# MaartenGr/PolyFuzz

Hardware: AMD Instinct MI355X
Metric: string-pairs/sec, TF-IDF cosine top-n 100k x 100k (config.timed_step says what a step is: by default the user-level .match() call of SURVEY section 8d's metric, `device_step` = the list resident in HBM; latency.top1_single_query_ms = top-1 match latency) (higher is better)
Workload: dtype f32

## Files before the change

### polyfuzz_amd/csrc/k1_vectorize.hip

```cpp
#include "pfz_internal.h"

#include <string.h>

#include <algorithm>
#include <atomic>
#include <type_traits>

namespace pfz {

constexpr uint32_t kInvalid = 0xFFFFFFFFu;
constexpr int kShortMax = 128;
constexpr int kLongMax = 4096;
constexpr int kLongTile = 16;
constexpr int kMaxCodeBits = 64;
constexpr int kBitmapMaxBits = 32;

static std::atomic<uint64_t> g_gen{1};

struct VocabView {
    const uint32_t *bitmap;
    const int32_t *prefix;
    const uint64_t *vcodes;
    int64_t vocab;
};
// ... 503 lines not shown
    df[k] = s;
}

constexpr int kHistRows = 1024;

__global__ __launch_bounds__(1024) void k_df_hist(const int64_t *__restrict__ off, int64_t n, int32_t R,
                                                   const uint64_t *__restrict__ slots,
                                                   const int32_t *__restrict__ row_nnz, int32_t words,
                                                   uint32_t *__restrict__ partial, ListB B = ListB{})
{
    __shared__ uint32_t h[kHistWords];
    for (int t = threadIdx.x; t < words; t += 1024) h[t] = 0u;
    __syncthreads();
    unsigned bx = blockIdx.x;
    if (bx >= B.grid0) {
        bx -= B.grid0;
        off = B.off;
        n = B.n;
        slots = B.slots;
        row_nnz = B.row_cnt + (B.n + 1);
    }
    const int64_t r0 = (int64_t)bx * kHistRows;
    const int64_t r1 = r0 + kHistRows < n ? r0 + kHistRows : n;
    const int grp = threadIdx.x >> 4, sub = threadIdx.x & 15;
    const int lane0 = (threadIdx.x & 63) & ~15;
    for (int64_t rb = r0 + grp * 16; rb < r1; rb += 64 * 16) {
        const int64_t mine = rb + sub;
        int nn = 0;
        int64_t so = 0;
        if (mine < r1) {
            nn = row_nnz[mine];
            so = off[mine] * R;
        }
        uint32_t kk[16];
        int nni[16];
#pragma unroll
        for (int i = 0; i < 16; ++i) {
            nni[i] = __shfl(nn, lane0 + i, 64);
            const int64_t soi = ((int64_t)__shfl((int)(so >> 32), lane0 + i, 64) << 32) |
                                (uint32_t)__shfl((int)(uint32_t)so, lane0 + i, 64);
            kk[i] = sub < nni[i] ? ((const uint2 *)(slots + soi))[sub].x : 0u;
        }
#pragma unroll
        for (int i = 0; i < 16; ++i)
            if (sub < nni[i]) atomicAdd(&h[kk[i] >> 1], 1u << ((kk[i] & 1u) * 16));
        for (int i = 0; i < 16; ++i) {
            const int n_i = __shfl(nn, lane0 + i, 64);
            if (n_i <= 16) continue;
            const int64_t soi = ((int64_t)__shfl((int)(so >> 32), lane0 + i, 64) << 32) |
                                (uint32_t)__shfl((int)(uint32_t)so, lane0 + i, 64);
            const uint2 *in = (const uint2 *)(slots + soi);
            for (int t = sub + 16; t < n_i; t += 16) {
                const uint32_t k = in[t].x;
                atomicAdd(&h[k >> 1], 1u << ((k & 1u) * 16));
            }
        }
    }
    __syncthreads();
    uint32_t *dst = partial + (int64_t)blockIdx.x * words;
    for (int t = threadIdx.x; t < words; t += 1024) dst[t] = h[t];
}

__global__ __launch_bounds__(256) void k_df_hist_reduce(const uint32_t *__restrict__ partial, int32_t words,
                                                         int32_t chunks, int64_t vocab, int32_t *__restrict__ df,
                                                         double n_docs = 0.0, double *__restrict__ idf = nullptr)
{
    const int w = blockIdx.x * 256 + threadIdx.x;
    if (w >= words) return;
    int32_t lo = 0, hi = 0;
#pragma unroll 8
    for (int c = 0; c < chunks; ++c) {
        const uint32_t v = partial[(int64_t)c * words + w];
        lo += (int32_t)(v & 0xffffu);
        hi += (int32_t)(v >> 16);
    }
    df[2 * (int64_t)w] = lo;
    if (2 * (int64_t)w + 1 < vocab) df[2 * (int64_t)w + 1] = hi;
    if (idf) {
        idf[2 * (int64_t)w] = log((n_docs + 1.0) / ((double)lo + 1.0)) + 1.0;
        if (2 * (int64_t)w + 1 < vocab) idf[2 * (int64_t)w + 1] = log((n_docs + 1.0) / ((double)hi + 1.0)) + 1.0;
    }
}

__global__ __launch_bounds__(256) void k_rows_short(const int64_t *__restrict__ off, int64_t n, int32_t R,
                                                     VocabView V, uint64_t *__restrict__ slots,
                                                     const int32_t *__restrict__ row_cnt,
                                                     int32_t *__restrict__ row_nnz, DfSink df, ListB B = ListB{})
{
    const int lane = threadIdx.x & 63;
    unsigned bx = blockIdx.x;
    if (bx >= B.grid0) {
        bx -= B.grid0;
        off = B.off;
        n = B.n;
        slots = B.slots;
        row_cnt = B.row_cnt;
        row_nnz = B.row_cnt + (B.n + 1);
    }
    const int64_t row = (int64_t)bx * 4 + (threadIdx.x >> 6);
    if (row >= n) return;
    const int cnt = row_cnt[row];
    if (cnt > kShortMax) return;
    if (cnt == 0) {
        if (lane == 0) row_nnz[row] = 0;
        return;
    }
    rows_short_row(V, slots + off[row] * R, cnt, lane, row_nnz + row, row, df);
}

template <typename KEYS>
__device__ inline void rows_long_body(KEYS keys, int cnt, const VocabView &V, uint64_t *base, int32_t *row_nnz_out,
                                      DfSink df, int *sh_heads, int *sh_valid)
{
    const int lane = threadIdx.x & 63, wave = threadIdx.x >> 6;
    int npow2 = 128;
    while (npow2 < cnt) npow2 <<= 1;
    for (int t = threadIdx.x; t < npow2; t += 256) keys[t] = t < cnt ? vocab_rank(V, base[t]) : kInvalid;
    __syncthreads();
    for (int k = 2; k <= npow2; k <<= 1) {
        for (int j = k >> 1; j > 0; j >>= 1) {
            for (int t = threadIdx.x; t < npow2; t += 256) {
                const int x = t ^ j;
                if (x > t) {
                    const bool asc = (t & k) == 0;
                    const uint32_t a = keys[t], b = keys[x];
                    if ((a > b) == asc) {
                        keys[t] = b;
                        keys[x] = a;
                    }
                }
            }
            __syncthreads();
        }
    }
    uint2 *out = (uint2 *)base;
    if (wave == 0) {
        int nheads = 0, nvalid = 0;
        for (int c0 = 0; c0 < cnt; c0 += 64) {
            const int t = c0 + lane;
            uint32_t key = kInvalid, prev = kInvalid;
            if (t < cnt) key = keys[t];
            if (t > 0 && t < cnt) prev = keys[t - 1];
            const bool valid = key != kInvalid;
            const bool head = valid && (t == 0 || key != prev);
            const uint64_t H = __ballot(head);
            if (head) {
                out[nheads + __popcll(H & ((1ull << lane) - 1ull))] = make_uint2(key, (uint32_t)t);
                df.add(key, blockIdx.x);
            }
            nheads += __popcll(H);
            nvalid += __popcll(__ballot(valid));
        }
        if (lane == 0) {
            *sh_heads = nheads;
            *sh_valid = nvalid;
            *row_nnz_out = nheads;
        }
    }
    __syncthreads();
    const int nheads = *sh_heads, nvalid = *sh_valid;
    for (int c0 = 0; c0 < nheads; c0 += 256) {
        const int p = c0 + threadIdx.x;
        uint32_t tf = 0;
        if (p < nheads) tf = (p + 1 < nheads ? out[p + 1].y : (uint32_t)nvalid) - out[p].y;
        __syncthreads();
        if (p < nheads) out[p].y = tf;
        __syncthreads();
    }
}

__global__ __launch_bounds__(256) void k_rows_long(const int64_t *__restrict__ off, int64_t n, int32_t R, VocabView V,
                                                    uint64_t *__restrict__ slots,
                                                    const int32_t *__restrict__ row_cnt,
                                                    int32_t *__restrict__ row_nnz, DfSink df,
                                                    uint32_t *__restrict__ giant_scratch, int64_t giant_stride)
{
    __shared__ uint32_t lds_keys[kLongMax];
    __shared__ int sh_heads, sh_valid, n_long;
    __shared__ int long_rows[kLongTile];
    const int64_t n_tiles = (n + kLongTile - 1) / kLongTile;
    for (int64_t tile = blockIdx.x; tile < n_tiles; tile += gridDim.x) {
        if (threadIdx.x == 0) n_long = 0;
        __syncthreads();
        const int64_t mine = tile * kLongTile + threadIdx.x;
        if ((int)threadIdx.x < kLongTile && mine < n && row_cnt[mine] > kShortMax) long_rows[atomicAdd(&n_long, 1)] = (int)threadIdx.x;
        __syncthreads();
        const int m = n_long;
        for (int i = 0; i < m; ++i) {
            const int64_t row = tile * kLongTile + long_rows[i];
            const int cnt = row_cnt[row];
            uint64_t *base = slots + off[row] * R;
            if (cnt <= kLongMax)
                rows_long_body(&lds_keys[0], cnt, V, base, row_nnz + row, df, &sh_heads, &sh_valid);
            else
                rows_long_body(giant_scratch + (int64_t)blockIdx.x * giant_stride, cnt, V, base, row_nnz + row, df,
                               &sh_heads, &sh_valid);
            __syncthreads();
        }
        __syncthreads();
    }
}

__global__ __launch_bounds__(256) void k_idf(const int32_t *__restrict__ df, int64_t vocab, double n_docs,
                                              double *__restrict__ idf)
{
    const int64_t k = (int64_t)blockIdx.x * 256 + threadIdx.x;
    if (k >= vocab) return;
    idf[k] = log((n_docs + 1.0) / ((double)df[k] + 1.0)) + 1.0;
}

__device__ inline double shfl_f64(double v, int src_lane)
{
    const int lo = __shfl(__double2loint(v), src_lane, 64), hi = __shfl(__double2hiint(v), src_lane, 64);
    return __hiloint2double(hi, lo);
}

constexpr int64_t kSelfScanRows = 16384;
template <bool SELF_SCAN>
__global__ __launch_bounds__(256) void k_finalize(const int64_t *__restrict__ off, int64_t n, int32_t R,
                                                   const uint64_t *__restrict__ slots,
                                                   int32_t *__restrict__ indptr, const double *__restrict__ idf,
                                                   int32_t *__restrict__ indices, float *__restrict__ data,
                                                   const int32_t *__restrict__ row_nnz, int32_t *__restrict__ host_total)
{
    const int64_t row = ((int64_t)blockIdx.x * 256 + threadIdx.x) >> 4;
    const int sub = threadIdx.x & 15;
    const int lane0 = (threadIdx.x & 63) & ~15;
    const bool live = row < n;
    const uint2 *in = live ? (const uint2 *)(slots + off[row] * R) : nullptr;
    int o, nn;
    if (SELF_SCAN) {
        __shared__ int32_t s_part[4], s_cnt[16];
        const int64_t row0 = (int64_t)blockIdx.x * 16;
        int32_t acc = 0;
        for (int64_t t = threadIdx.x; t < row0; t += 256) acc += row_nnz[t];
        for (int d = 32; d >= 1; d >>= 1) acc += __shfl_xor(acc, d, 64);
        if ((threadIdx.x & 63) == 0) s_part[threadIdx.x >> 6] = acc;
        if (threadIdx.x < 16) s_cnt[threadIdx.x] = row0 + threadIdx.x < n ? row_nnz[row0 + threadIdx.x] : 0;
        __syncthreads();
        o = s_part[0] + s_part[1] + s_part[2] + s_part[3];
        const int mine = (int)(row - row0);
        for (int k = 0; k < mine; ++k) o += s_cnt[k];
        nn = live ? s_cnt[mine] : 0;
        if (live && sub == 0) indptr[row] = o;
        if (row == n - 1 && sub == 0) {
            indptr[n] = o + nn;
            if (host_total) __hip_atomic_store(host_total, o + nn, __ATOMIC_RELAXED, __HIP_MEMORY_SCOPE_SYSTEM);
        }
    } else {
        o = live ? indptr[row] : 0;
        nn = live ? indptr[row + 1] - o : 0;
    }
    int nn_max = nn;
    for (int d = 16; d < 64; d <<= 1) nn_max = max(nn_max, __shfl_xor(nn_max, d, 64));
    double ss = 0.0;
    for (int c0 = 0; c0 < nn_max; c0 += 16) {
        const int t = c0 + sub;
        double v = 0.0;
        if (t < nn) {
            const uint2 e = in[t];
            v = __dmul_rn((double)e.y, idf[e.x]);
        }
        const double v2 = __dmul_rn(v, v);
        const int m = min(16, nn_max - c0);
        for (int j = 0; j < m; ++j) {
            const double term = shfl_f64(v2, lane0 + j);
            if (c0 + j < nn) ss = __dadd_rn(ss, term);
        }
    }
    const double nrm = sqrt(ss);
    for (int t = sub; t < nn; t += 16) {
        const uint2 e = in[t];
        double v = __dmul_rn((double)e.y, idf[e.x]);
        if (ss != 0.0) v = v / nrm;
        indices[o + t] = (int32_t)e.x;
        data[o + t] = (float)v;
    }
}

__global__ __launch_bounds__(256) void k_copy_i32(const int32_t *__restrict__ src, int64_t n, int32_t *__restrict__ dst)
{
    const int64_t i = (int64_t)blockIdx.x * 256 + threadIdx.x;
    if (i < n) dst[i] = src[i];
}

static inline unsigned grid_for(int64_t n, int per_block = 256) { return (unsigned)((n + per_block - 1) / per_block); }

static int bits_for(uint64_t max_value)
{
    int b = 1;
    while ((max_value >> b) != 0) ++b;
    return b;
}

static int prepare_slots(pfz_ctx *ctx, const pfz_tfidf *v, pfz_strings *s)
{
    const int R = v->params.ngram_hi - v->params.ngram_lo + 1;
    const size_t need = (size_t)(s->n_units > 0 ? s->n_units : 1) * (size_t)R;
    if (s->slots_cap < need) {
        if (s->slots) pool_free(s->slots);
        s->slots = nullptr;
        PFZ_TRY(pool_alloc(ctx, &s->slots, need * sizeof(uint64_t)));
        s->slots_cap = need;
    }
    if (!s->row_cnt) PFZ_TRY(pool_alloc(ctx, &s->row_cnt, (size_t)(s->n + 1) * 2 * sizeof(int32_t)));
    return PFZ_OK;
}

static int run_extract(pfz_ctx *ctx, const pfz_tfidf *v, pfz_strings *s, bool mark, bool *rows_done = nullptr,
                       pfz_strings *sb = nullptr, bool *sb_done = nullptr)
{
    if (sb_done) *sb_done = false;
    PFZ_TRY(prepare_slots(ctx, v, s));
    if (s->n == 0) return PFZ_OK;
    const int64_t bitmap_words = v->n_groups * 8;
    ExtractParams P{v->params.ngram_lo, v->params.ngram_hi, v->params.clean, v->params.remove_space_ngrams,
                    v->bits_per_char, (int32_t)(bitmap_words <= kLdsBitmapWords ? bitmap_words : 0), v->alpha_map_len};
    const bool lds_bitmap = mark && bitmap_words <= kLdsBitmapWords;
    ProfScope ps(ctx, "k1_extract");
    const char *which = getenv("PFZ_K1_EXTRACT");
    const bool wave = s->max_len <= kWaveMaxLen && (which ? which[0] == 'w' : s->n <= 32768);
    int per_wg = 32;
    if (const char *e = getenv("PFZ_K1_WAVE_STRINGS")) per_wg = std::max(4, std::min(kWaveStringsMax, atoi(e)));
    ListB B;
    unsigned grid_b = 0;
    const char *two_knob = getenv("PFZ_K1_TWO_LISTS");
    if (sb && sb_done && wave && sb->n > 0 && sb->n <= 32768 && sb->max_len <= kWaveMaxLen && sb->char_width == s->char_width &&
        !(which && which[0] != 'w') && !(two_knob && atoi(two_knob) == 0)) {
        PFZ_TRY(prepare_slots(ctx, v, sb));
        B.chars = sb->chars;
        B.off = sb->offsets;
        B.n = sb->n;
        B.slots = sb->slots;
        B.row_cnt = sb->row_cnt;
        B.grid0 = grid_for(s->n, per_wg);
        grid_b = grid_for(sb->n, per_wg);
        *sb_done = true;
    }
    const char *fuse_knob = getenv("PFZ_K1_FUSE_ROWS");
    if (rows_done) *rows_done = false;
    if (rows_done && !mark && wave && !(fuse_knob && atoi(fuse_knob) == 0)) {
        VocabView V{v->bitmap, v->prefix, v->vcodes, v->vocab};
        int32_t *row_nnz = s->row_cnt + (s->n + 1);
#define PFZ_EXTRACT_ROWS(CW, CODE)                                                                                   \
        hipLaunchKernelGGL((k_extract_wave<CW, false, CODE, true>), dim3(grid_for(s->n, per_wg)), dim3(256), 0, ctx->stream,      \
                           s->chars, s->offsets, s->n, P, v->alpha_map, s->slots, s->row_cnt, nullptr, per_wg, V, row_nnz)
        if (s->char_width == 1) {
            if (v->code_bits <= 32) PFZ_EXTRACT_ROWS(1, uint32_t);
            else PFZ_EXTRACT_ROWS(1, uint64_t);
        } else {
            if (v->code_bits <= 32) PFZ_EXTRACT_ROWS(4, uint32_t);
            else PFZ_EXTRACT_ROWS(4, uint64_t);
        }
#undef PFZ_EXTRACT_ROWS
        PFZ_HIP(hipGetLastError());
        *rows_done = true;
        return PFZ_OK;
    }
#define PFZ_EXTRACT(CW, LB)                                                                                          \
    do {                                                                                                             \
        if (wave && v->code_bits <= 32)                                                                              \
            hipLaunchKernelGGL((k_extract_wave<CW, LB, uint32_t>), dim3(grid_for(s->n, per_wg) + grid_b), dim3(256), 0,       \
                               ctx->stream, s->chars, s->offsets, s->n, P, v->alpha_map, s->slots, s->row_cnt,       \
                               mark ? v->bitmap : nullptr, per_wg, VocabView{}, nullptr, B);                         \
        else if (wave)                                                                                               \
            hipLaunchKernelGGL((k_extract_wave<CW, LB, uint64_t>), dim3(grid_for(s->n, per_wg) + grid_b), dim3(256), 0,       \
                               ctx->stream, s->chars, s->offsets, s->n, P, v->alpha_map, s->slots, s->row_cnt,       \
                               mark ? v->bitmap : nullptr, per_wg, VocabView{}, nullptr, B);                         \
        else if (v->code_bits <= 32)                                                                                 \
            hipLaunchKernelGGL((k_extract<CW, LB, uint32_t>), dim3(grid_for(s->n)), dim3(256), 0, ctx->stream,       \
                               s->chars, s->offsets, s->n, P, v->alpha_map, s->slots, s->row_cnt,                    \
                               mark ? v->bitmap : nullptr);                                                          \
        else                                                                                                         \
            hipLaunchKernelGGL((k_extract<CW, LB, uint64_t>), dim3(grid_for(s->n)), dim3(256), 0, ctx->stream,       \
                               s->chars, s->offsets, s->n, P, v->alpha_map, s->slots, s->row_cnt,                    \
                               mark ? v->bitmap : nullptr);                                                          \
    } while (0)
    if (s->char_width == 1) {
        if (lds_bitmap) PFZ_EXTRACT(1, true);
        else PFZ_EXTRACT(1, false);
    } else {
        if (lds_bitmap) PFZ_EXTRACT(4, true);
        else PFZ_EXTRACT(4, false);
    }
#undef PFZ_EXTRACT
    PFZ_HIP(hipGetLastError());
    return PFZ_OK;
}

static int run_rows(pfz_ctx *ctx, const pfz_tfidf *v, pfz_strings *s, DfSink df, bool short_done = false, pfz_strings *sb = nullptr)
{
    if (s->n == 0) return sb ? run_rows(ctx, v, sb, df) : PFZ_OK;
    const int R = v->params.ngram_hi - v->params.ngram_lo + 1;
    VocabView V{v->bitmap, v->prefix, v->vcodes, v->vocab};
    int32_t *row_nnz = s->row_cnt + (s->n + 1);
    if (!short_done) {
        ListB B;
        unsigned grid_b = 0;
        if (sb && sb->n > 0) {
            B.off = sb->offsets;
            B.n = sb->n;
            B.slots = sb->slots;
            B.row_cnt = sb->row_cnt;
            B.grid0 = grid_for(s->n, 4);
            grid_b = grid_for(sb->n, 4);
        }
        ProfScope ps(ctx, "k2_rows_short");
        hipLaunchKernelGGL(k_rows_short, dim3(grid_for(s->n, 4) + grid_b), dim3(256), 0, ctx->stream, s->offsets, s->n, R, V,
                           s->slots, s->row_cnt, row_nnz, df, B);
    }
    if (s->max_len * R > kShortMax) {
        const int64_t max_cnt = s->max_len * R;
        const int64_t n_tiles = (s->n + kLongTile - 1) / kLongTile;
        unsigned grid = (unsigned)std::min<int64_t>(n_tiles, 2048);
        uint32_t *giant = nullptr;
        int64_t stride = 0;
        if (max_cnt > kLongMax) {
            grid = (unsigned)std::min<int64_t>(n_tiles, 64);
            stride = 128;
            while (stride < max_cnt) stride <<= 1;
            PFZ_TRY(ensure_scratch(ctx, (size_t)grid * (size_t)stride * sizeof(uint32_t)));
            giant = (uint32_t *)ctx->scratch;
        }
        ProfScope ps(ctx, "k2_rows_long");
        hipLaunchKernelGGL(k_rows_long, dim3(grid), dim3(256), 0, ctx->stream, s->offsets, s->n, R, V, s->slots,
                           s->row_cnt, row_nnz, df, giant, stride);
    }
    PFZ_HIP(hipGetLastError());
    if (sb && !short_done) return run_rows(ctx, v, sb, df, true);
    return PFZ_OK;
}

static int build_prefix(pfz_ctx *ctx, pfz_tfidf *v, LazyI32 *size)
{
    if (v->n_groups >= 1 && v->n_groups <= 1024) {
        if (size) PFZ_TRY(lazy_acquire(ctx, size));
        hipLaunchKernelGGL(k_group_popc_scan, dim3(1), dim3(1024), 0, ctx->stream, v->bitmap, (int32_t)v->n_groups, v->prefix,
                           size ? size->slot : nullptr);
        PFZ_HIP(hipGetLastError());
        return size ? lazy_mark(ctx, size) : PFZ_OK;
    }
    hipLaunchKernelGGL(k_group_popc, dim3(grid_for(v->n_groups)), dim3(256), 0, ctx->stream, v->bitmap, v->n_groups,
                       v->prefix);
    return exclusive_scan_i32(ctx, v->prefix, v->n_groups, size);
}

static int64_t vocab_bound(int64_t a, int lo, int hi)
{
    int64_t total = 0, p = 1;
    for (int n = 1; n <= hi; ++n) {
        if (p > ((int64_t)1 << 40) / (a > 0 ? a : 1)) return (int64_t)1 << 40;
        p *= a;
        if (n >= lo) total += p;
    }
    return total;
}

static int build_sorted_vocab(pfz_ctx *ctx, pfz_tfidf *v, pfz_strings *const lists[2])
{
    const int R = v->params.ngram_hi - v->params.ngram_lo + 1;
    struct Tmp {
        void *p = nullptr;
        ~Tmp() { if (p) pool_free(p); }
    } code_off[2], gathered, sorted, flags;
    int64_t base[2] = {0, 0}, total = 0;
    for (int li = 0; li < 2; ++li) {
        pfz_strings *s = lists[li];
        if (!s || s->n == 0) continue;
        PFZ_TRY(pool_alloc(ctx, &code_off[li].p, (size_t)(s->n + 1) * sizeof(int32_t)));
        hipLaunchKernelGGL(k_copy_i32, dim3(grid_for(s->n)), dim3(256), 0, ctx->stream, s->row_cnt, s->n, (int32_t *)code_off[li].p);
        PFZ_TRY(exclusive_scan_i32(ctx, (int32_t *)code_off[li].p, s->n));
        int32_t t = 0;
        PFZ_HIP(hipMemcpyAsync(&t, (int32_t *)code_off[li].p + s->n, sizeof(int32_t), hipMemcpyDeviceToHost, ctx->stream));
        PFZ_HIP(hipStreamSynchronize(ctx->stream));
        base[li] = total;
        total += t;
    }
    v->vocab = 0;
    if (total == 0) return PFZ_OK;
    if (total >= ((int64_t)1 << 31) - 2) {
        set_error("pfz_tfidf_fit: %lld n-gram occurrences exceed the int32 layout of the sorted-vocabulary path", (long long)total);
        return PFZ_ERR_UNSUPPORTED;
    }
    PFZ_TRY(pool_alloc(ctx, &gathered.p, (size_t)total * sizeof(uint64_t)));
    PFZ_TRY(pool_alloc(ctx, &sorted.p, (size_t)sort_codes_capacity(total) * sizeof(uint64_t)));
    PFZ_TRY(pool_alloc(ctx, &flags.p, (size_t)(total + 1) * sizeof(int32_t)));
    for (int li = 0; li < 2; ++li) {
        pfz_strings *s = lists[li];
        if (!s || s->n == 0) continue;
        hipLaunchKernelGGL(k_gather_codes, dim3(grid_for(s->n, 16)), dim3(256), 0, ctx->stream, s->offsets, s->n, R, s->slots,
                           (const int32_t *)code_off[li].p, (uint64_t *)gathered.p + base[li]);
    }
    PFZ_TRY(sort_codes_u64(ctx, (const uint64_t *)gathered.p, (uint64_t *)sorted.p, total));
    hipLaunchKernelGGL(k_flag_heads, dim3(grid_for(total)), dim3(256), 0, ctx->stream, (const uint64_t *)sorted.p, total,
                       (int32_t *)flags.p);
    PFZ_TRY(exclusive_scan_i32(ctx, (int32_t *)flags.p, total));
    int32_t n_distinct = 0;
    PFZ_HIP(hipMemcpyAsync(&n_distinct, (int32_t *)flags.p + total, sizeof(int32_t), hipMemcpyDeviceToHost, ctx->stream));
    PFZ_HIP(hipStreamSynchronize(ctx->stream));
    PFZ_TRY(pool_alloc(ctx, &v->vcodes, (size_t)n_distinct * sizeof(uint64_t)));
    hipLaunchKernelGGL(k_scatter_heads, dim3(grid_for(total)), dim3(256), 0, ctx->stream, (const uint64_t *)sorted.p, total,
                       (const int32_t *)flags.p, v->vcodes);
    PFZ_HIP(hipGetLastError());
    v->vocab = n_distinct;
    return PFZ_OK;
}

static int merge_sorted_vocab(pfz_ctx *ctx, pfz_comm *comm, pfz_tfidf *v)
{
    const int world = comm_world(comm);
    struct Tmp {
        void *p = nullptr;
        ~Tmp() { if (p) pool_free(p); }
    } sizes, send, gathered, sorted, flags;
    PFZ_TRY(pool_alloc(ctx, &sizes.p, (size_t)(world + 1) * sizeof(int64_t)));
    const int64_t mine = v->vocab;
    PFZ_TRY(copy_h2d(ctx, (int64_t *)sizes.p + world, &mine, sizeof(int64_t)));
    PFZ_TRY(comm_allgather_bytes(comm, (int64_t *)sizes.p + world, sizes.p, sizeof(int64_t)));
    std::vector<int64_t> h((size_t)world);
    PFZ_TRY(copy_d2h(ctx, h.data(), sizes.p, (size_t)world * sizeof(int64_t)));
    int64_t longest = 0, total = 0;
    for (int64_t x : h) {
        longest = std::max(longest, x);
        total += x;
    }
    Tmp old_codes;
    old_codes.p = v->vcodes;
    v->vcodes = nullptr;
    v->vocab = 0;
    if (total == 0) return PFZ_OK;
    if ((int64_t)world * longest >= ((int64_t)1 << 31) - 2) {
        set_error("pfz_tfidf_fit_sharded: %lld distinct n-grams per rank exceed the int32 layout of the sorted-vocabulary path",
                  (long long)longest);
        return PFZ_ERR_UNSUPPORTED;
    }
    const int64_t padded = (int64_t)world * longest;
    PFZ_TRY(pool_alloc(ctx, &send.p, (size_t)longest * sizeof(uint64_t)));
    PFZ_HIP(hipMemsetAsync(send.p, 0xff, (size_t)longest * sizeof(uint64_t), ctx->stream));
    if (mine > 0) PFZ_HIP(hipMemcpyAsync(send.p, old_codes.p, (size_t)mine * sizeof(uint64_t), hipMemcpyDeviceToDevice, ctx->stream));
    PFZ_TRY(pool_alloc(ctx, &gathered.p, (size_t)padded * sizeof(uint64_t)));
    PFZ_TRY(comm_allgather_bytes(comm, send.p, gathered.p, (size_t)longest * sizeof(uint64_t)));
    PFZ_TRY(pool_alloc(ctx, &sorted.p, (size_t)sort_codes_capacity(padded) * sizeof(uint64_t)));
    PFZ_TRY(pool_alloc(ctx, &flags.p, (size_t)(total + 1) * sizeof(int32_t)));
    PFZ_TRY(sort_codes_u64(ctx, (const uint64_t *)gathered.p, (uint64_t *)sorted.p, padded));
    hipLaunchKernelGGL(k_flag_heads, dim3(grid_for(total)), dim3(256), 0, ctx->stream, (const uint64_t *)sorted.p, total,
                       (int32_t *)flags.p);
    PFZ_TRY(exclusive_scan_i32(ctx, (int32_t *)flags.p, total));
    int32_t n_distinct = 0;
    PFZ_TRY(copy_d2h(ctx, &n_distinct, (int32_t *)flags.p + total, sizeof(int32_t)));
    PFZ_TRY(pool_alloc(ctx, &v->vcodes, (size_t)n_distinct * sizeof(uint64_t)));
    hipLaunchKernelGGL(k_scatter_heads, dim3(grid_for(total)), dim3(256), 0, ctx->stream, (const uint64_t *)sorted.p, total,
                       (const int32_t *)flags.p, v->vcodes);
    PFZ_HIP(hipGetLastError());
    v->vocab = n_distinct;
// ... 324 lines not shown
        hipError_t e = hipMemcpyAsync(d_n, &local_docs, sizeof(int64_t), hipMemcpyHostToDevice, ctx->stream);
        int rc = PFZ_OK;
        if (e == hipSuccess) rc = comm_allreduce_sum_i64(comm, d_n, 1);
        int64_t total = 0;
        if (e == hipSuccess && rc == PFZ_OK) e = hipMemcpyAsync(&total, d_n, sizeof(int64_t), hipMemcpyDeviceToHost, ctx->stream);
        if (e == hipSuccess && rc == PFZ_OK) e = hipStreamSynchronize(ctx->stream);
        pool_free(d_n);
        PFZ_TRY(rc);
        PFZ_HIP(e);
        v->n_docs = total;
    }
    if (!idf_fused)
        hipLaunchKernelGGL(k_idf, dim3(grid_for(v->vocab)), dim3(256), 0, ctx->stream, v->df, v->vocab, (double)v->n_docs,
                           v->idf);
    PFZ_HIP(hipGetLastError());
    guard.p = nullptr;
    *out = v;
    return PFZ_OK;
}

extern "C" {

int pfz_tfidf_fit(pfz_ctx *ctx, const pfz_tfidf_params *params, const pfz_strings *docs_a, const pfz_strings *docs_b,
                  pfz_tfidf **out)
{
    return fit_impl(ctx, nullptr, params, docs_a, docs_b, out);
}

int pfz_tfidf_fit_sharded(pfz_ctx *ctx, pfz_comm *comm, const pfz_tfidf_params *params, const pfz_strings *replicated,
                          const pfz_strings *local_shard, pfz_tfidf **out)
{
    PFZ_REQUIRE(comm, "pfz_tfidf_fit_sharded: NULL communicator");
    PFZ_REQUIRE(replicated != local_shard || !replicated, "pfz_tfidf_fit_sharded: the replicated and the sharded list must differ");
    return fit_impl(ctx, comm, params, replicated, local_shard, out);
}

int pfz_tfidf_info(const pfz_tfidf *v, int64_t *vocab_size, int64_t *n_docs, int32_t *code_bits)
{
    PFZ_REQUIRE(v, "pfz_tfidf_info: NULL vectoriser");
    if (vocab_size) *vocab_size = v->vocab;
    if (n_docs) *n_docs = v->n_docs;
    if (code_bits) *code_bits = v->code_bits;
    return PFZ_OK;
}

int pfz_tfidf_transform(pfz_ctx *ctx, const pfz_tfidf *v, const pfz_strings *docs_c, pfz_csr **out)
{
    PFZ_REQUIRE(ctx && v && docs_c && out, "pfz_tfidf_transform: NULL argument");
    PFZ_HIP(hipSetDevice(ctx->device));
    pfz_strings *s = const_cast<pfz_strings *>(docs_c);
    if (v->params.clean && s->char_width != 1) {
        set_error("pfz_tfidf_transform: clean=1 runs on 1-byte code units only; pre-clean wide strings on the host");
        return PFZ_ERR_INVALID;
    }
    if (s->cache_gen != v->gen) {
        bool rows_done = false;
        PFZ_TRY(run_extract(ctx, v, s, false, &rows_done));
        PFZ_TRY(run_rows(ctx, v, s, DfSink{nullptr, 0}, rows_done));
        s->cache_gen = v->gen;
    }
    const int R = v->params.ngram_hi - v->params.ngram_lo + 1;
    Owner<pfz_csr, pfz_csr_free> m(new pfz_csr());
    m->ctx = ctx;
    m->n_rows = s->n;
    m->n_cols = v->vocab;
    PFZ_TRY(pool_alloc(ctx, &m->indptr, (size_t)(s->n + 1) * sizeof(int32_t)));
    const int64_t cap = std::max<int64_t>(1, std::min<int64_t>(s->n_units * (int64_t)R, ((int64_t)1 << 31) - 1));
    m->nnz_cap = cap;
    PFZ_TRY(pool_alloc(ctx, &m->indices, (size_t)cap * sizeof(int32_t)));
    PFZ_TRY(pool_alloc(ctx, &m->data, (size_t)cap * sizeof(float)));
    if (s->n > 0) {
        const int32_t *row_nnz = s->row_cnt + (s->n + 1);
        const char *knob = getenv("PFZ_K2_SELF_SCAN");
        const bool no_self_scan = knob && atoi(knob) == 0;
        if (s->n <= kSelfScanRows && !no_self_scan) {
            PFZ_TRY(lazy_acquire(ctx, &m->nnz_lazy));
            {
                ProfScope ps(ctx, "k2_finalize");
                hipLaunchKernelGGL(k_finalize<true>, dim3(grid_for(s->n, 16)), dim3(256), 0, ctx->stream, s->offsets, s->n, R, s->slots,
                                   m->indptr, v->idf, m->indices, m->data, row_nnz, m->nnz_lazy.slot);
            }
            PFZ_TRY(lazy_mark(ctx, &m->nnz_lazy));
        } else {
            hipLaunchKernelGGL(k_copy_i32, dim3(grid_for(s->n)), dim3(256), 0, ctx->stream, row_nnz, s->n, m->indptr);
            PFZ_TRY(exclusive_scan_i32(ctx, m->indptr, s->n, &m->nnz_lazy));
            ProfScope ps(ctx, "k2_finalize");
            hipLaunchKernelGGL(k_finalize<false>, dim3(grid_for(s->n, 16)), dim3(256), 0, ctx->stream, s->offsets, s->n, R, s->slots,
                               m->indptr, v->idf, m->indices, m->data, nullptr, nullptr);
        }
    } else {
        PFZ_HIP(hipMemsetAsync(m->indptr, 0, sizeof(int32_t), ctx->stream));
        m->nnz = 0;
    }
    PFZ_HIP(hipGetLastError());
    *out = m.release();
    return PFZ_OK;
}

int pfz_tfidf_export(pfz_ctx *ctx, const pfz_tfidf *v, uint32_t *ngrams, double *idf, int64_t *df)
{
    PFZ_REQUIRE(ctx && v, "pfz_tfidf_export: NULL argument");
    PFZ_HIP(hipSetDevice(ctx->device));
    PFZ_HIP(hipStreamSynchronize(ctx->stream));
    if (idf && v->vocab > 0) PFZ_HIP(hipMemcpy(idf, v->idf, (size_t)v->vocab * sizeof(double), hipMemcpyDeviceToHost));
    if (df && v->vocab > 0) {
        std::vector<int32_t> h((size_t)v->vocab);
        PFZ_HIP(hipMemcpy(h.data(), v->df, h.size() * sizeof(int32_t), hipMemcpyDeviceToHost));
        for (size_t i = 0; i < h.size(); ++i) df[i] = h[i];
    }
    if (ngrams && v->vocab > 0) {
        std::vector<uint64_t> codes((size_t)v->vocab);
        if (v->vcodes) {
            PFZ_HIP(hipMemcpy(codes.data(), v->vcodes, codes.size() * sizeof(uint64_t), hipMemcpyDeviceToHost));
        } else {
            uint64_t *d_codes = nullptr;
            PFZ_TRY(pool_alloc(ctx, &d_codes, (size_t)v->vocab * sizeof(uint64_t)));
            hipLaunchKernelGGL(k_export_codes, dim3(grid_for(v->n_groups)), dim3(256), 0, ctx->stream, v->bitmap, v->prefix,
                               v->n_groups, d_codes);
            hipError_t e = hipMemcpyAsync(codes.data(), d_codes, codes.size() * sizeof(uint64_t), hipMemcpyDeviceToHost, ctx->stream);
            if (e == hipSuccess) e = hipStreamSynchronize(ctx->stream);
            pool_free(d_codes);
            PFZ_HIP(e);
        }
        const int hi = v->params.ngram_hi, w = v->bits_per_char;
        const uint64_t cmask = (1ull << w) - 1ull;
        for (size_t i = 0; i < codes.size(); ++i)
            for (int p = 0; p < hi; ++p) {
                const uint32_t m = (uint32_t)((codes[i] >> ((hi - 1 - p) * w)) & cmask);
                uint32_t cp = 0;
                if (m != 0) cp = v->params.clean ? clean_rank_to_cp(m) : v->alphabet[m - 1];
                ngrams[i * hi + p] = cp;
            }
    }
    return PFZ_OK;
}

int pfz_tfidf_import(pfz_ctx *ctx, const pfz_tfidf_params *params, int64_t vocab, int64_t n_docs, const uint32_t *ngrams,
                     const double *idf, pfz_tfidf **out)
{
    PFZ_REQUIRE(ctx && out && ngrams && idf && vocab > 0, "pfz_tfidf_import: bad arguments");
    PFZ_TRY(check_params(params));
    PFZ_HIP(hipSetDevice(ctx->device));
    pfz_tfidf *v = new pfz_tfidf();
    struct Guard {
        pfz_tfidf *p;
        ~Guard() { if (p) pfz_tfidf_free(p); }
    } guard{v};
    v->ctx = ctx;
    v->params = *params;
    v->gen = g_gen.fetch_add(1);
    v->n_docs = n_docs;
    const int hi = params->ngram_hi;
    if (params->clean) {
        v->bits_per_char = 6;
        v->code_bits = 6 * hi;
        if (v->code_bits > kMaxCodeBits) {
            set_error("pfz_tfidf_import: %d-grams of cleaned strings exceed the %d-bit code space", hi, kMaxCodeBits);
            return PFZ_ERR_UNSUPPORTED;
        }
    } else {
        std::vector<uint32_t> cps;
        for (int64_t i = 0; i < vocab * hi; ++i)
            if (ngrams[i]) cps.push_back(ngrams[i]);
        std::sort(cps.begin(), cps.end());
        cps.erase(std::unique(cps.begin(), cps.end()), cps.end());
        PFZ_TRY(set_alphabet(ctx, v, cps));
    }
    const int w = v->bits_per_char;
// ... 55 lines not shown
```

### polyfuzz_amd/csrc/k3_cossim_topn.hip

```cpp
#include "k3_core.h"

#include <algorithm>
#include <math.h>
#include <stdlib.h>

namespace pfz {

constexpr int kMergeCap = 256;
constexpr int kMaxTop = 1024;

__global__ __launch_bounds__(256) void k_index_count(const int32_t *__restrict__ indptr,
                                                      const int32_t *__restrict__ indices, int32_t n_rows,
                                                      int32_t nb, int32_t block, int32_t *__restrict__ cnt)
{
    const int gid = (blockIdx.x * 256 + threadIdx.x) >> 4;
    const int sub = threadIdx.x & 15;
    if (gid >= n_rows) return;
    const int p0 = indptr[gid], p1 = indptr[gid + 1];
    const int b = gid / block;
    for (int p = p0 + sub; p < p1; p += 16) atomicAdd(&cnt[(int64_t)indices[p] * nb + b], 1);
}

__global__ __launch_bounds__(256) void k_index_fill(const int32_t *__restrict__ indptr,
                                                     const int32_t *__restrict__ indices,
                                                     const float *__restrict__ data, int32_t n_rows, int32_t nb,
                                                     int32_t block, int32_t *__restrict__ cnt,
                                                     const int32_t *__restrict__ tab, int2 *__restrict__ post)
{
    const int gid = (blockIdx.x * 256 + threadIdx.x) >> 4;
    const int sub = threadIdx.x & 15;
    if (gid >= n_rows) return;
    const int p0 = indptr[gid], p1 = indptr[gid + 1];
    const int b = gid / block;
    const int local = gid - b * block;
    for (int p = p0 + sub; p < p1; p += 16) {
        const int64_t slot = (int64_t)indices[p] * nb + b;
        const int pos = atomicSub(&cnt[slot], 1) - 1;
        post[(int64_t)tab[slot] * kPiece + pos] = make_int2(local * 4, __float_as_int(data[p]));
    }
}

constexpr int kSub = 4;
__global__ __launch_bounds__(256) void k_index_pieces(int32_t *__restrict__ cnt, int32_t *__restrict__ sub, int64_t slots,
                                                       int32_t *__restrict__ tab, int32_t *__restrict__ heavy, int32_t heavy_cap,
                                                       int32_t bank_min)
{
    const int64_t i = (int64_t)blockIdx.x * 256 + threadIdx.x;
    int c = 0;
    if (i == 0) tab[-1] = 1;
    if (i < slots) {
        if (sub) {
            int4 v = ((const int4 *)sub)[i];
            c = v.x + v.y + v.z + v.w;
            if (c) ((int4 *)sub)[i] = make_int4(0, v.x, v.x + v.y, v.x + v.y + v.z);
            cnt[i] = c;
        } else {
            c = cnt[i];
        }
        tab[i] = (c + kPiece - 1) / kPiece;
    } else if (i < slots + 2) {
        tab[i] = 0;
    }
    const bool h = heavy && i < slots && c >= bank_min;
    const uint64_t m = __ballot(h);
    if (m) {
        const int lane = threadIdx.x & 63, first = __ffsll((long long)m) - 1;
        int base = 0;
        if (lane == first) base = atomicAdd(&heavy[0], __popcll(m));
        base = __shfl(base, first, 64);
        const int at = base + __popcll(m & ((1ull << lane) - 1ull));
        if (h && at < heavy_cap) heavy[1 + at] = (int32_t)i;
    }
}

__global__ __launch_bounds__(256) void k_index_pad(const int32_t *__restrict__ cnt, const int32_t *__restrict__ tab,
                                                    int64_t slots, int2 *__restrict__ post,
                                                    uint16_t *__restrict__ pblk, int32_t nb, const int32_t *__restrict__ nnz_dev,
                                                    int32_t *__restrict__ nnz_host)
{
    const int64_t i = (int64_t)blockIdx.x * 256 + threadIdx.x;
    if (i == 0) __hip_atomic_store(nnz_host, *nnz_dev, __ATOMIC_RELAXED, __HIP_MEMORY_SCOPE_SYSTEM);
    if (i < kPiece) post[i] = make_int2((int)i * 4, 0);
    if (i == 0 && pblk) pblk[0] = 0;
    if (i >= slots) return;
    const int c = cnt[i];
    if (c == 0) return;
    if (pblk) {
        const uint16_t b = (uint16_t)((uint32_t)i % (uint32_t)nb);
        const int first = tab[i], last = first + (c + kPiece - 1) / kPiece;
        for (int p = first; p < last; ++p) pblk[p] = b;
    }
    if ((c & (kPiece - 1)) == 0) return;
    const int64_t base = (int64_t)tab[i] * kPiece;
    const int end = (c + kPiece - 1) & ~(kPiece - 1);
    for (int p = c; p < end; ++p) post[base + p] = make_int2(((((int)i & 3) << 4) | (p & 15)) * 4, 0);
}

__global__ __launch_bounds__(1024) void k_index_count_lds(const int32_t *__restrict__ indptr,
                                                           const int32_t *__restrict__ indices, int32_t n_rows,
                                                           int32_t nb, int32_t block, int32_t words,
                                                           int32_t *__restrict__ sub_cnt )
{
    __shared__ uint32_t h[kHistWords];
    for (int t = threadIdx.x; t < words; t += 1024) h[t] = 0u;
    __syncthreads();
    const int b = blockIdx.x / kSub, q = blockIdx.x % kSub;
    const int per = block / kSub;
    const int lo = b * block + q * per, hi = min(n_rows, lo + per);
    const int grp = threadIdx.x >> 4, sub = threadIdx.x & 15;
    const int lane0 = (threadIdx.x & 63) & ~15;
    for (int rb = lo + grp * 16; rb < hi; rb += 64 * 16) {
        const int mine = rb + sub;
        int q0 = 0, q1 = 0;
        if (mine < hi) {
            q0 = indptr[mine];
            q1 = indptr[mine + 1];
        }
        int kk[16], p0i[16], p1i[16];
#pragma unroll
        for (int i = 0; i < 16; ++i) {
            p0i[i] = __shfl(q0, lane0 + i, 64);
            p1i[i] = __shfl(q1, lane0 + i, 64);
            kk[i] = p0i[i] + sub < p1i[i] ? indices[p0i[i] + sub] : 0;
        }
#pragma unroll
        for (int i = 0; i < 16; ++i)
            if (p0i[i] + sub < p1i[i]) atomicAdd(&h[kk[i] >> 1], 1u << ((kk[i] & 1) * 16));
        for (int i = 0; i < 16; ++i) {
            const int a = __shfl(q0, lane0 + i, 64), e = __shfl(q1, lane0 + i, 64);
            for (int p = a + 16 + sub; p < e; p += 16) {
                const int k = indices[p];
                atomicAdd(&h[k >> 1], 1u << ((k & 1) * 16));
            }
        }
    }
    __syncthreads();
    for (int w = threadIdx.x; w < words; w += 1024) {
        const uint32_t v = h[w];
        if (v & 0xffffu) sub_cnt[((int64_t)(2 * w) * nb + b) * kSub + q] = (int32_t)(v & 0xffffu);
        if (v >> 16) sub_cnt[((int64_t)(2 * w + 1) * nb + b) * kSub + q] = (int32_t)(v >> 16);
    }
}

__global__ __launch_bounds__(1024) void k_index_fill_lds(const int32_t *__restrict__ indptr,
                                                          const int32_t *__restrict__ indices,
                                                          const float *__restrict__ data, int32_t n_rows, int32_t nb,
                                                          int32_t block, int32_t words,
                                                          const int32_t *__restrict__ tab ,
                                                          const int32_t *__restrict__ sub_first ,
                                                          int2 *__restrict__ post)
{
    __shared__ uint32_t h[kHistWords];
    for (int t = threadIdx.x; t < words; t += 1024) h[t] = 0u;
    __syncthreads();
    const int b = blockIdx.x / kSub, q = blockIdx.x % kSub;
    const int per = block / kSub;
    const int blk0 = b * block;
    const int lo = blk0 + q * per, hi = min(n_rows, lo + per);
    const int grp = threadIdx.x >> 4, sub = threadIdx.x & 15;
    const int lane0 = (threadIdx.x & 63) & ~15;
    auto place = [&](int k, float v, int row, int64_t start) {
        const int sh = (k & 1) * 16;
        const uint32_t old = atomicAdd(&h[k >> 1], 1u << sh);
        post[start + (int)((old >> sh) & 0xffffu)] = make_int2((row - blk0) * 4, __float_as_int(v));
    };
    auto start_of = [&](int k) -> int64_t {
        const int64_t slot = (int64_t)k * nb + b;
        return (int64_t)tab[slot] * kPiece + sub_first[slot * kSub + q];
    };
    for (int rb = lo + grp * 16; rb < hi; rb += 64 * 16) {
        const int mine = rb + sub;
        int q0 = 0, q1 = 0;
        if (mine < hi) {
            q0 = indptr[mine];
            q1 = indptr[mine + 1];
        }
        int kk[16];
        int64_t st[16];
        float vv[16];
        bool ok[16];
#pragma unroll
        for (int i = 0; i < 16; ++i) {
            const int a = __shfl(q0, lane0 + i, 64), e = __shfl(q1, lane0 + i, 64);
            ok[i] = a + sub < e;
            kk[i] = ok[i] ? indices[a + sub] : 0;
            vv[i] = ok[i] ? data[a + sub] : 0.f;
        }
#pragma unroll
        for (int i = 0; i < 16; ++i) st[i] = ok[i] ? start_of(kk[i]) : 0;
#pragma unroll
        for (int i = 0; i < 16; ++i)
            if (ok[i]) place(kk[i], vv[i], rb + i, st[i]);
        for (int i = 0; i < 16; ++i) {
            const int a = __shfl(q0, lane0 + i, 64), e = __shfl(q1, lane0 + i, 64);
            for (int p = a + 16 + sub; p < e; p += 16) {
                const int k = indices[p];
                place(k, data[p], rb + i, start_of(k));
            }
        }
    }
}

template <int C, int kCap, bool kBounded = false>
__global__ __launch_bounds__(64) void k3_cossim_topn_kernel(
    const int32_t *__restrict__ a_indptr, const int32_t *__restrict__ a_idx, const float *__restrict__ a_val,
    int32_t n_a, const int32_t *__restrict__ tab, const int2 *__restrict__ post, int32_t nb, int32_t n_pieces,
    int32_t ntop, int32_t thr0, float scale, float inv_scale, int32_t exclude_diag, int64_t diag_offset,
    int32_t *__restrict__ out_idx, float *__restrict__ out_val, int32_t ablate, int32_t n_slices,
    uint64_t *__restrict__ part_keys, uint64_t *__restrict__ ub = nullptr)
{
    __shared__ __attribute__((aligned(16))) struct {
        int acc[C];
        uint64_t cand[kCap];
    } sm;
    static_assert(kCap >= 64 + 32, "the last 32 keys of the candidate buffer double as the scatter's marker scratch");
    int *const acc = sm.acc;
    uint64_t *const cand = sm.cand;
    int *const mark = (int *)(sm.cand + kCap) - 64;
    if ((uint32_t)(uintptr_t)sm.acc != 0u) __builtin_trap();
    const int lane = threadIdx.x;
    int4 *acc4 = (int4 *)acc;
    constexpr int N4 = C / 4;
    int zero;
    asm volatile("v_mov_b32 %0, 0" : "=v"(zero));
    for (int t = lane; t < C / 4; t += 64) acc4[t] = make_int4(0, 0, 0, 0);
    wave_sync();
    const char *post_bytes = (const char *)post;
    const int src4 = (4 * (lane & 15) + (lane >> 4)) * 4;
    const int sub8 = (lane & 15) * 8;
    const int dummy_addr = 0;
    (void)n_pieces;

    const int per_slice = (nb + n_slices - 1) / n_slices;
    for (int item = blockIdx.x; item < n_a * n_slices; item += gridDim.x) {
        const int row = item / n_slices, slice = item - row * n_slices;
        const int b_lo = slice * per_slice, b_hi = min(nb, b_lo + per_slice);
        const int p0 = a_indptr[row], p1 = a_indptr[row + 1];
        const int nnz = p1 - p0;
        const int64_t self_col64 = (int64_t)row + diag_offset;
        const int self_col = (exclude_diag && self_col64 >= 0 && self_col64 < 0x7fffffff) ? (int)self_col64 : -1;
        TopState st;
        st.cnt = 0;
        st.thr = thr0;

        const int n_blk = b_hi - b_lo;
        int b_first = b_lo;
#if PFZ_K3_EXP != 8
        if (self_col >= 0 && self_col / C >= b_lo && self_col / C < b_hi) b_first = self_col / C;
#endif
        int cur0 = 0, nxt0 = 0;
        float as0 = 0.f;
        const bool have0 = lane < nnz;
        const int32_t *trow = tab;
        if (have0) {
            as0 = a_val[p0 + lane] * scale;
            trow = tab + (int64_t)a_idx[p0 + lane] * nb;
            cur0 = trow[b_first];
            nxt0 = trow[b_first + 1];
        }

        bool warmed = ablate == 3 || kBounded;
        const uint64_t ub_row = kBounded ? ub[row] : ~0ull;
        for (int it = 0, b = b_first; it < n_blk; ++it) {
            const int s = cur0, e = have0 ? nxt0 : cur0;
            const int b_next = b + 1 < b_hi ? b + 1 : b_lo;
            bool touched = __ballot(e > s) != 0;
            if (touched && ablate != 1) scatter_pieces(acc, post_bytes, mark, e - s, s, as0, lane, src4, sub8, dummy_addr);
            if (have0 && it + 1 < n_blk) {
                cur0 = trow[b_next];
                nxt0 = trow[b_next + 1];
            }
            for (int c0 = p0 + 64; c0 < p1; c0 += 64) {
                int s2 = 0, e2 = 0;
                float as2 = 0.f;
                if (c0 + lane < p1) {
                    const int k = a_idx[c0 + lane];
                    as2 = a_val[c0 + lane] * scale;
                    s2 = tab[(int64_t)k * nb + b];
                    e2 = tab[(int64_t)k * nb + b + 1];
                }
                if (__ballot(e2 > s2)) {
                    touched = true;
                    scatter_pieces(acc, post_bytes, mark, e2 - s2, s2, as2, lane, src4, sub8, dummy_addr);
                }
            }
            if (touched && ablate != 2) {
                wave_sync();
                if (!warmed) {
                    warmed = true;
                    if (ntop <= kWarmMaxTop) {
                        const int t = warm_threshold<N4>(acc4, 0, ntop + (self_col >= 0 ? 1 : 0), lane);
                        st.thr = t > st.thr ? t : st.thr;
                    }
                }
                sweep_block<N4, kCap, kBounded>(acc4, cand, st, b * C, self_col, ntop, lane, zero, ub_row);
                wave_sync();
            }
            b = b_next;
        }

        compact<kCap>(cand, st, ntop, lane);
        if (kBounded && lane == 0) ub[row] = st.cnt == ntop ? cand[ntop - 1] : 0ull;
        for (int r = lane; r < ntop; r += 64) {
            const uint64_t key = r < st.cnt ? cand[r] : 0ull;
            if (n_slices > 1) {
                part_keys[((int64_t)row * n_slices + slice) * ntop + r] = key;
            } else {
                out_idx[(int64_t)row * ntop + r] = key ? (int32_t)(~(uint32_t)key) : -1;
                out_val[(int64_t)row * ntop + r] = key ? (float)(int32_t)(uint32_t)(key >> 32) * inv_scale : 0.f;
            }
        }
        wave_sync();
    }
}

constexpr int kBankMin = 64, kBankCap = 1024;
__global__ __launch_bounds__(256) void k_index_bank_order(const int32_t *__restrict__ cnt, const int32_t *__restrict__ tab,
                                                           const int32_t *__restrict__ heavy, int32_t heavy_cap,
                                                           int2 *__restrict__ post)
{
    __shared__ int2 s_buf[4][kBankCap];
    __shared__ int s_cnt[4][32];
    const int lane = threadIdx.x & 63, wave = threadIdx.x >> 6;
    int2 *buf = s_buf[wave];
    int *bc = s_cnt[wave];
    const int n_heavy = min(heavy[0], heavy_cap);
    const int n_waves = (int)gridDim.x * 4;
    for (int h = (int)blockIdx.x * 4 + wave; h < n_heavy; h += n_waves) {
        {
            const int64_t slot = heavy[1 + h];
            const int c = min(cnt[slot], kBankCap);
            const int64_t base = (int64_t)tab[slot] * kPiece;
            if (lane < 32) bc[lane] = 0;
            __builtin_amdgcn_fence(__ATOMIC_ACQ_REL, "wavefront");
            __builtin_amdgcn_wave_barrier();
            for (int i = lane; i < c; i += 64) {
                int2 pe = post[base + i];
                const int b = (pe.x >> 2) & 31;
                const int j = atomicAdd(&bc[b], 1);
                buf[i] = make_int2(pe.x, pe.y);
                buf[i].x = pe.x | (j << 16);
            }
            __builtin_amdgcn_fence(__ATOMIC_ACQ_REL, "wavefront");
            __builtin_amdgcn_wave_barrier();
            const int my_cnt = lane < 32 ? bc[lane] : 0;
            for (int i = lane; i < c + 63 - (c + 63) % 64; i += 64) {
                const bool on = i < c;
                int2 pe = on ? buf[i] : make_int2(0, 0);
                const int j = (int)((uint32_t)pe.x >> 16), b = (pe.x >> 2) & 31;
                int pos = 0;
#pragma unroll
                for (int q = 0; q < 32; ++q) {
                    const int cq = __shfl(my_cnt, q, 64);
                    pos += min(cq, j) + ((q < b && cq > j) ? 1 : 0);
                }
                if (on) post[base + pos] = make_int2(pe.x & 0xffff, pe.y);
            }
            __builtin_amdgcn_fence(__ATOMIC_ACQ_REL, "wavefront");
            __builtin_amdgcn_wave_barrier();
        }
    }
}

__global__ __launch_bounds__(256) void k3_merge_slices(const uint64_t *__restrict__ part_keys, int32_t n_a,
                                                       int32_t n_slices, int32_t ntop, float inv_scale,
                                                       int32_t *__restrict__ out_idx, float *__restrict__ out_val)
{
    constexpr int kCap = kMergeCap;
    __shared__ __attribute__((aligned(16))) uint64_t cand_all[4][kCap];
    const int lane = threadIdx.x & 63, wave = threadIdx.x >> 6;
    const int row = blockIdx.x * 4 + wave;
    if (row >= n_a) return;
    uint64_t *cand = cand_all[wave];
    TopState st;
    st.cnt = 0;
    st.thr = 0;
    const uint64_t *src = part_keys + (int64_t)row * n_slices * ntop;
    const int total = n_slices * ntop;
    for (int e0 = 0; e0 < total; e0 += 64) {
        const uint64_t key = e0 + lane < total ? src[e0 + lane] : 0ull;
        const uint64_t mk = __ballot(key != 0ull);
        if (key) cand[st.cnt + __popcll(mk & ((1ull << lane) - 1ull))] = key;
        st.cnt += __popcll(mk);
        if (st.cnt > kCap - 64) compact<kCap>(cand, st, ntop, lane, false);
    }
    compact<kCap>(cand, st, ntop, lane);
    for (int r = lane; r < ntop; r += 64) {
        const uint64_t key = r < st.cnt ? cand[r] : 0ull;
        out_idx[(int64_t)row * ntop + r] = key ? (int32_t)(~(uint32_t)key) : -1;
        out_val[(int64_t)row * ntop + r] = key ? (float)(int32_t)(uint32_t)(key >> 32) * inv_scale : 0.f;
    }
}

__global__ __launch_bounds__(256) void k_topn_place(const int32_t *__restrict__ t_idx, const float *__restrict__ t_val, int64_t n_rows,
                                                    int32_t w, int32_t ntop, int32_t col0, int32_t *__restrict__ out_idx,
                                                    float *__restrict__ out_val)
{
    const int64_t i = (int64_t)blockIdx.x * 256 + threadIdx.x;
    if (i >= n_rows * w) return;
    const int64_t r = i / w;
    const int c = (int)(i - r * w);
    out_idx[r * ntop + col0 + c] = t_idx[i];
    out_val[r * ntop + col0 + c] = t_val[i];
}

static int env_int(const char *name, int dflt)
{
    const char *v = getenv(name);
    return v && *v ? atoi(v) : dflt;
}

int index_ready(const pfz_index *ix)
{
    int32_t v = 0;
    if (ix->pieces_lazy.pending) {
        PFZ_TRY(lazy_get(ix->ctx, &ix->pieces_lazy, &v));
        ix->n_pieces = v - 1;
    }
    if (ix->nnz_lazy.pending) {
        PFZ_TRY(lazy_get(ix->ctx, &ix->nnz_lazy, &v));
        ix->nnz = v;
    }
    return PFZ_OK;
}

}

using namespace pfz;

extern "C" {

int pfz_index_build(pfz_ctx *ctx, const pfz_csr *B, pfz_index **out)
{
    PFZ_REQUIRE(ctx && B && out, "pfz_index_build: NULL argument");
    PFZ_HIP(hipSetDevice(ctx->device));
    int block = env_int("PFZ_K3_BLOCK", 2048);
    if (block != 1024 && block != 1536 && block != 2048 && block != 4096) block = 2048;
    const int64_t nb = (B->n_rows + block - 1) / block;
    const int64_t slots = B->n_cols * nb;
    if (slots >= ((int64_t)1 << 31) - 2) {
        set_error("pfz_index_build: vocabulary %lld x %lld to-blocks exceeds the int32 offset table",
                  (long long)B->n_cols, (long long)nb);
        return PFZ_ERR_UNSUPPORTED;
    }
    Owner<pfz_index, pfz_index_free> ix(new pfz_index());
    ix->ctx = ctx;
    ix->n_rows = B->n_rows;
    ix->n_cols = B->n_cols;
    ix->block_cols = block;
    ix->n_blocks = (int32_t)nb;
    ix->max_norm = B->max_norm;
    ix->src_serial = B->serial;
    struct Tmp {
        int32_t *p = nullptr;
        ~Tmp() { if (p) pool_free(p); }
    } cnt, sub;
    const bool any = B->n_rows > 0;
    const bool lds_hist = B->n_cols <= 2 * (int64_t)kHistWords && !getenv("PFZ_NO_LDS_HIST");
    PFZ_TRY(pool_alloc(ctx, &ix->tab_base, (size_t)(slots + 3) * sizeof(int32_t)));
    ix->tab = ix->tab_base + 1;
    PFZ_TRY(pool_alloc(ctx, &cnt.p, (size_t)(slots + 2) * sizeof(int32_t)));
    if (lds_hist && any) {
        PFZ_TRY(pool_alloc(ctx, &sub.p, (size_t)(slots + 1) * kSub * sizeof(int32_t)));
        PFZ_HIP(hipMemsetAsync(sub.p, 0, (size_t)slots * kSub * sizeof(int32_t), ctx->stream));
    } else {
        PFZ_HIP(hipMemsetAsync(cnt.p, 0, (size_t)(slots + 2) * sizeof(int32_t), ctx->stream));
    }
    const char *bo_env = getenv("PFZ_K3_BANK_ORDER");
    const bool bank_order = any && lds_hist && !getenv("PFZ_K3_NO_BANK_ORDER") &&
                            ((bo_env && atoi(bo_env) > 0) || (!bo_env && B->n_rows >= 32768));
    const int32_t bank_min = kBankMin;
    const int32_t heavy_cap = (int32_t)std::min<int64_t>(slots, (int64_t)1 << 22);
    Tmp heavy;
    if (bank_order) {
        PFZ_TRY(pool_alloc(ctx, &heavy.p, (size_t)(heavy_cap + 1) * sizeof(int32_t)));
        PFZ_HIP(hipMemsetAsync(heavy.p, 0, sizeof(int32_t), ctx->stream));
    }
    const int32_t words = (int32_t)((B->n_cols + 1) / 2);
    const unsigned row_grid = (unsigned)((B->n_rows * 16 + 255) / 256);
    const unsigned slot_grid = (unsigned)((slots + kPiece + 255) / 256);
    {
        ProfScope ps(ctx, "k_index_count");
        if (any && lds_hist)
            hipLaunchKernelGGL(k_index_count_lds, dim3((unsigned)nb * kSub), dim3(1024), 0, ctx->stream, B->indptr, B->indices,
                               (int32_t)B->n_rows, (int32_t)nb, block, words, sub.p);
        else if (any)
            hipLaunchKernelGGL(k_index_count, dim3(row_grid), dim3(256), 0, ctx->stream, B->indptr, B->indices,
                               (int32_t)B->n_rows, (int32_t)nb, block, cnt.p);
        hipLaunchKernelGGL(k_index_pieces, dim3(slot_grid), dim3(256), 0, ctx->stream, cnt.p, lds_hist && any ? sub.p : nullptr, slots,
                           ix->tab, heavy.p, heavy_cap, bank_min);
    }
    PFZ_TRY(exclusive_scan_i32(ctx, ix->tab_base, slots + 1, &ix->pieces_lazy));
    const int64_t nnz_bound = B->nnz_lazy.pending ? B->nnz_cap : B->nnz;
    int64_t piece_cap = nnz_bound / kPiece + std::min<int64_t>(slots, nnz_bound) + 1;
    if (piece_cap > kPieceBoundMax) {
        int32_t total = 0;
        PFZ_TRY(lazy_get(ctx, &ix->pieces_lazy, &total));
        ix->n_pieces = total - 1;
        if (total - 1 >= (1 << 25) - 1) {
            set_error("pfz_index_build: %d index pieces (%lld postings padded to 16 per list and block) exceed the 4 GiB "
                      "the kernel addresses with 32-bit byte offsets", total - 1, (long long)csr_nnz(B));
            return PFZ_ERR_UNSUPPORTED;
        }
        piece_cap = total;
    }
    ix->piece_cap = piece_cap;
    PFZ_TRY(lazy_acquire(ctx, &ix->nnz_lazy));
    PFZ_TRY(pool_alloc(ctx, &ix->post, (size_t)piece_cap * kPiece * sizeof(int2)));
    if (block == 2048 && nb >= 2 && nb < 65536)
        PFZ_TRY(pool_alloc(ctx, &ix->pblk, (size_t)piece_cap * sizeof(uint16_t)));
    {
        ProfScope ps(ctx, "k_index_fill");
        hipLaunchKernelGGL(k_index_pad, dim3(slot_grid), dim3(256), 0, ctx->stream, cnt.p, ix->tab, slots, ix->post, ix->pblk, (int32_t)nb,
                           B->indptr + B->n_rows, ix->nnz_lazy.slot);
        PFZ_TRY(lazy_mark(ctx, &ix->nnz_lazy));
        if (any && lds_hist)
            hipLaunchKernelGGL(k_index_fill_lds, dim3((unsigned)nb * kSub), dim3(1024), 0, ctx->stream, B->indptr, B->indices,
                               B->data, (int32_t)B->n_rows, (int32_t)nb, block, words, ix->tab, sub.p, ix->post);
        else if (any)
            hipLaunchKernelGGL(k_index_fill, dim3(row_grid), dim3(256), 0, ctx->stream, B->indptr, B->indices, B->data,
                               (int32_t)B->n_rows, (int32_t)nb, block, cnt.p, ix->tab, ix->post);
    }
    if (bank_order) {
        ProfScope ps(ctx, "k_index_bank_order");
        hipLaunchKernelGGL(k_index_bank_order, dim3((unsigned)ctx->prop.multiProcessorCount * 4), dim3(256), 0, ctx->stream, cnt.p,
                           ix->tab, heavy.p, heavy_cap, ix->post);
    }
    PFZ_HIP(hipGetLastError());
    *out = ix.release();
    return PFZ_OK;
}

void pfz_index_free(pfz_index *ix)
{
    if (!ix) return;
    if (ix->ctx) (void)hipSetDevice(ix->ctx->device);
    k3_sym_free(ix);
    for (LazyI32 *z : {&ix->pieces_lazy, &ix->nnz_lazy})
        if (z->pending || z->slot) {
            if (z->ev) (void)hipEventSynchronize(z->ev);
            lazy_release(ix->ctx, z);
        }
    if (ix->tab_base) pool_free(ix->tab_base);
    if (ix->post) pool_free(ix->post);
    if (ix->pblk) pool_free(ix->pblk);
    delete ix;
}

int pfz_index_info(const pfz_index *ix, int64_t *n_rows, int64_t *n_cols, int64_t *nnz, int64_t *block_cols,
                   int64_t *n_blocks, int64_t *table_bytes)
{
    PFZ_REQUIRE(ix, "pfz_index_info: NULL index");
    PFZ_TRY(index_ready(ix));
    if (n_rows) *n_rows = ix->n_rows;
    if (n_cols) *n_cols = ix->n_cols;
    if (nnz) *nnz = ix->nnz;
    if (block_cols) *block_cols = ix->block_cols;
    if (n_blocks) *n_blocks = ix->n_blocks;
    if (table_bytes) *table_bytes = (ix->n_cols * ix->n_blocks + 2) * (int64_t)sizeof(int32_t);
    return PFZ_OK;
}

int pfz_index_pieces(const pfz_index *ix, int64_t *n_pieces, int64_t *piece_postings)
{
    PFZ_REQUIRE(ix, "pfz_index_pieces: NULL index");
    PFZ_TRY(index_ready(ix));
    if (n_pieces) *n_pieces = ix->n_pieces;
    if (piece_postings) *piece_postings = kPiece;
    return PFZ_OK;
}

int pfz_cossim_topn(pfz_ctx *ctx, const pfz_index *ix, const pfz_csr *A, int32_t ntop, float lower_bound,
                    int32_t exclude_diag, int64_t diag_offset, pfz_topn *out)
{
    PFZ_REQUIRE(A, "pfz_cossim_topn: NULL argument");
    return pfz_cossim_topn_rows(ctx, ix, A, 0, A->n_rows, ntop, lower_bound, exclude_diag, diag_offset, out);
}

int pfz_cossim_topn_rows(pfz_ctx *ctx, const pfz_index *ix, const pfz_csr *A, int64_t row_begin, int64_t row_end,
                         int32_t ntop, float lower_bound, int32_t exclude_diag, int64_t diag_offset, pfz_topn *out)
{
    PFZ_REQUIRE(ctx && ix && A && out, "pfz_cossim_topn: NULL argument");
    PFZ_REQUIRE(row_begin >= 0 && row_begin <= row_end && row_end <= A->n_rows,
                "pfz_cossim_topn_rows: rows [%lld, %lld) outside [0, %lld)", (long long)row_begin, (long long)row_end,
                (long long)A->n_rows);
    PFZ_REQUIRE(ntop >= 1, "pfz_cossim_topn: ntop must be >= 1 (got %d)", ntop);
    PFZ_REQUIRE(A->n_cols == ix->n_cols, "pfz_cossim_topn: from-matrix has %lld columns, index has %lld",
                (long long)A->n_cols, (long long)ix->n_cols);
    PFZ_REQUIRE(out->n_rows >= A->n_rows && out->ntop == ntop, "pfz_cossim_topn: result buffer is %lldx%d, need %lldx%d",
                (long long)out->n_rows, out->ntop, (long long)A->n_rows, ntop);
    PFZ_REQUIRE(lower_bound == lower_bound, "pfz_cossim_topn: lower_bound is NaN");
    const int64_t n_rows = row_end - row_begin;
    if (n_rows == 0) return PFZ_OK;
    PFZ_HIP(hipSetDevice(ctx->device));
    float scale, inv_scale;
    int32_t thr0;
    k3_fixed_point(A, ix, lower_bound, &scale, &inv_scale, &thr0);
    if (ntop > kMaxTop) {
        struct Tmp {
            void *p = nullptr;
            ~Tmp() { if (p) pool_free(p); }
        } t_idx, t_val, ub;
        PFZ_TRY(pool_alloc(ctx, &t_idx.p, (size_t)n_rows * kMaxTop * sizeof(int32_t)));
        PFZ_TRY(pool_alloc(ctx, &t_val.p, (size_t)n_rows * kMaxTop * sizeof(float)));
        PFZ_TRY(pool_alloc(ctx, &ub.p, (size_t)n_rows * sizeof(uint64_t)));
        PFZ_HIP(hipMemsetAsync(ub.p, 0xff, (size_t)n_rows * sizeof(uint64_t), ctx->stream));
        const int64_t max_grid = (int64_t)ctx->prop.multiProcessorCount * 16 * 64 * 8;
        const unsigned grid = (unsigned)(n_rows < max_grid ? n_rows : max_grid);
        ProfScope ps(ctx, "k3_cossim_topn");
        for (int32_t col0 = 0; col0 < ntop; col0 += kMaxTop) {
            const int32_t w = ntop - col0 < kMaxTop ? ntop - col0 : kMaxTop;
#define PFZ_K3_DEEP(CC)                                                                                                   \
    hipLaunchKernelGGL((k3_cossim_topn_kernel<CC, 1152, true>), dim3(grid), dim3(64), 0, ctx->stream, A->indptr + row_begin,     \
                       A->indices, A->data, (int32_t)n_rows, ix->tab, ix->post, ix->n_blocks, 0, w, thr0, scale,      \
                       inv_scale, exclude_diag, diag_offset + row_begin, (int32_t *)t_idx.p, (float *)t_val.p, 0, 1,              \
                       (uint64_t *)nullptr, (uint64_t *)ub.p)
            switch (ix->block_cols) {
            case 1024: PFZ_K3_DEEP(1024); break;
            case 1536: PFZ_K3_DEEP(1536); break;
            case 2048: PFZ_K3_DEEP(2048); break;
            case 4096: PFZ_K3_DEEP(4096); break;
            default:
                set_error("pfz_cossim_topn: no kernel for block size %d", ix->block_cols);
// ... 173 lines not shown
```

### polyfuzz_amd/csrc/k3_symmetric.hip

```cpp
#include "k3_core.h"

#include <stdio.h>
#include <stdlib.h>

namespace pfz {

constexpr int kSymC = 2048;
constexpr int kSymCap = 96;
constexpr int kSymKeep = 32;
#ifndef PFZ_K3_SYM_F
#define PFZ_K3_SYM_F 128
#endif
#ifndef PFZ_K3_SYM_PUSH
#define PFZ_K3_SYM_PUSH 512
#endif
constexpr int kSymF = PFZ_K3_SYM_F;
constexpr int kSymPush = PFZ_K3_SYM_PUSH;
constexpr int kSymMergeCap = kSymPush + 64;
#ifndef PFZ_K3_SYM_SIDE_STREAMS
#define PFZ_K3_SYM_SIDE_STREAMS 2
#endif
constexpr int kSymSides = PFZ_K3_SYM_SIDE_STREAMS;
static_assert(kSymSides >= 1 && kSymSides <= 4, "one to four side streams");
constexpr int kSymSlices = 8;
constexpr int kSymSlicedRows = 4096;
#ifndef PFZ_K3_SYM_EXP
#define PFZ_K3_SYM_EXP 0
#endif
constexpr int kSymMag = 1;
constexpr int kSymMagBlocks = 8;
constexpr int kSymP0PerCu = 128;
constexpr int kSymDoneStride = 32;
constexpr int kNoThr = 0x7fffffff;

struct K3SymArgs {
    const int32_t *a_indptr;
    const int32_t *a_idx;
    const float *a_val;
    int32_t n;
    const int32_t *tab;
    const int2 *post;
    const int2 *post_sym;
    const uint16_t *pblk;
    const int32_t *n_pieces1;
    int32_t nb, ntop, thr0;
    float scale, inv_scale;
    int32_t row_begin, row_end;
    int32_t n_parts, my_part, per;
    int32_t thr_by_part;
    uint64_t *keys_out;
    int32_t *thrv;
    uint16_t *slot4;
    uint32_t *gmin;
    int32_t *thr_slot;
    uint16_t *row_slot;
    int32_t *mag;
    int32_t n_mag_items, mag_b0, mag_row_end;
    uint64_t *keys;
    int32_t *push_cnt;
    uint64_t *push_buf;
    int32_t *ovf;
    uint64_t *part;
    int32_t ovf_base, ovf_max, n_sl;
    int32_t *out_idx;
    float *out_val;
    int32_t *host_idx;
    float *host_val;
    uint32_t *done;
    int32_t blk_lo, blk_hi;
};

__device__ inline int thr_pos(const K3SymArgs &a, int row)
{
    return a.thr_by_part ? (row % a.n_parts) * a.per + row / a.n_parts : row;
}
__device__ inline bool row_is_mine(const K3SymArgs &a, int row) { return a.n_parts == 1 || row % a.n_parts == a.my_part; }


__host__ __device__ inline int sym_slot(int rho, int i, int *t, int *l, int *e)
{
    const int p = i >> 1, half = i & 1, c = rho & 3;
    *t = p >> 3;
    *l = (rho >> 2) + 8 * (p & 7);
    *e = half * 4 + c;
    return 512 * *t + 256 * half + 4 * *l + c;
}

__global__ __launch_bounds__(1024) void k3_sym_order(const K3SymArgs a)
{
    __shared__ int s_gmin[256];
    const int b = blockIdx.x, lane = threadIdx.x & 63, wave = threadIdx.x >> 6;
    if (threadIdx.x < 256) s_gmin[threadIdx.x] = kNoThr;
    if (threadIdx.x == 0 && a.done) a.done[b * kSymDoneStride] = 0u;
    __syncthreads();
    for (int rho = wave * 2; rho < wave * 2 + 2; ++rho) {
        const int r = rho + 32 * lane;
        const int row = b * kSymC + r;
        if (row < a.n) a.push_cnt[row] = 0;
        const int thr = row < a.n ? a.thrv[thr_pos(a, row)] : kNoThr;
        const uint64_t key = ((uint64_t)(uint32_t)thr << 6) | (uint32_t)lane;
        int rank = 0;
#pragma unroll 16
        for (int m = 0; m < 64; ++m) {
            const uint32_t lo = (uint32_t)__builtin_amdgcn_readlane((int)(uint32_t)key, m);
            const uint32_t hi = (uint32_t)__builtin_amdgcn_readlane((int)(uint32_t)(key >> 32), m);
            rank += ((((uint64_t)hi << 32) | lo) < key) ? 1 : 0;
        }
        int t, l, e;
        const int slot = sym_slot(rho, rank, &t, &l, &e);
        const bool magnet = rank < kSymMag && row < a.n && b > 0;
        if (rank < kSymMag) a.mag[(int64_t)b * (32 * kSymMag) + rho * kSymMag + rank] = magnet ? row : -1;
        a.slot4[(int64_t)b * kSymC + r] = (uint16_t)(slot * 4);
        a.thr_slot[(int64_t)b * kSymC + slot] = magnet ? kNoThr : thr;
        a.row_slot[(int64_t)b * kSymC + slot] = (uint16_t)r;
        if (!magnet) atomicMin(&s_gmin[t * 64 + l], thr);
    }
    __syncthreads();
    if (threadIdx.x < 64) {
        uint32_t w = 0;
        for (int t = 0; t < 4; ++t) {
            const int g = s_gmin[t * 64 + threadIdx.x];
            w |= (g == kNoThr ? 0xffu : (uint32_t)g >> 24) << (8 * t);
        }
        a.gmin[(int64_t)b * 64 + threadIdx.x] = w;
    }
}

__global__ __launch_bounds__(256) void k3_sym_repost(const K3SymArgs a)
{
    const int64_t i = (int64_t)blockIdx.x * 256 + threadIdx.x;
    if (i >= (int64_t)*a.n_pieces1 * (kPiece / 2)) return;
    const int piece = (int)(i >> 3);
    const int b = a.pblk[piece];
    int4 e = ((const int4 *)a.post)[i];
    const uint16_t *s4 = a.slot4 + (int64_t)b * kSymC;
    if (piece > 0) {
        e.x = s4[e.x >> 2];
        e.z = s4[e.z >> 2];
    }
    ((int4 *)a.post_sym)[i] = e;
}


constexpr uint32_t kStageOwn = 1u << 30;
constexpr uint32_t kStageFgn = 1u << 31;

#ifndef PFZ_K3_SYM_PLAIN_STORES
#define PFZ_K3_SYM_PLAIN_STORES 0
#endif
__device__ inline void store_coherent(uint64_t *p, uint64_t v)
{
#if PFZ_K3_SYM_PLAIN_STORES
    *p = v;
#else
    __hip_atomic_store(p, v, __ATOMIC_RELAXED, __HIP_MEMORY_SCOPE_AGENT);
#endif
}

__device__ inline void sym_item_done(const K3SymArgs &a, int blk, int lane)
{
    if (!a.done) return;
    asm volatile("s_waitcnt vmcnt(0)" ::: "memory");
    if (lane == 0) __hip_atomic_fetch_add(&a.done[blk * kSymDoneStride], 1u, __ATOMIC_RELAXED, __HIP_MEMORY_SCOPE_AGENT);
}

__device__ inline uint32_t sym_items_of_block(const K3SymArgs &a, int b)
{
    const int rows = b < a.nb - 1 ? (a.n - b * kSymC < kSymC ? a.n - b * kSymC : kSymC) : 0;
    return (uint32_t)(rows + 32 * kSymMag * ((a.nb - 1 + kSymMagBlocks - 1) / kSymMagBlocks));
}

__global__ __launch_bounds__(64) void k3_sym_wait(const K3SymArgs a, int32_t *flag, int32_t flag_value)
{
    const int lane = threadIdx.x;
    if (lane == 0) {
        if (flag) __hip_atomic_store(flag, flag_value, __ATOMIC_RELAXED, __HIP_MEMORY_SCOPE_SYSTEM);
// ... 480 lines not shown
{
    K3SymState *s = ix->sym;
    if (!s) return;
    void *const bufs[] = {s->thrv, s->slot4, s->gmin, s->thr_slot, s->row_slot, s->mag, s->post_sym, s->keys, s->push_cnt, s->push_buf, s->ovf, s->part, s->ovfx[0], s->partx[0], s->ovfx[1], s->partx[1], s->ovfx[2], s->partx[2], s->done};
    for (void *p : bufs)
        if (p) pool_free(p);
    delete s;
    ix->sym = nullptr;
}

static int sym_env_int(const char *name, int dflt)
{
    const char *v = getenv(name);
    return v && *v ? atoi(v) : dflt;
}

int k3_sym_wanted(const pfz_ctx *ctx, const pfz_index *ix, const pfz_csr *A, int64_t row_begin, int64_t row_end, int32_t ntop,
                  int32_t thr0, float scale, int32_t exclude_diag, int64_t diag_offset, const pfz_topn *out)
{
    (void)ctx;
    const int force = sym_env_int("PFZ_K3_SYM", -1);
    if (force == 0) return 0;
    if (!exclude_diag || diag_offset != 0 || A->serial != ix->src_serial || A->n_rows != ix->n_rows) return 0;
    if (ix->block_cols != kSymC || !ix->pblk || ntop > kSymKeep || ix->n_blocks < 2 || ix->n_rows >= ((int64_t)1 << 30)) return 0;
    const K3SymState *s = ix->sym;
    if (s && s->n < 0) return 0;
    if (row_begin > 0) {
        const bool cont = s && s->next_row == row_begin && s->a_serial == A->serial && s->out == out && s->ntop == ntop &&
                          s->thr0 == thr0 && s->scale == scale;
        return cont ? 2 : 0;
    }
    if (force == 1) return 1;
    if (ix->n_rows < sym_env_int("PFZ_K3_SYM_MIN", 20480) || ix->n_rows > 250000) return 0;
    return (row_end - row_begin) * 5 >= ix->n_rows ? 1 : 0;
}

static int sym_state_alloc(pfz_ctx *ctx, const pfz_index *ix, K3SymState *s)
{
    const int64_t n = ix->n_rows;
    const size_t cells = (size_t)ix->n_blocks * kSymC;
    PFZ_TRY(pool_alloc(ctx, &s->thrv, (size_t)(n + 64) * sizeof(int32_t)));
    PFZ_TRY(pool_alloc(ctx, &s->slot4, cells * sizeof(uint16_t)));
    PFZ_TRY(pool_alloc(ctx, &s->gmin, cells / 32 * sizeof(uint32_t)));
    PFZ_TRY(pool_alloc(ctx, &s->thr_slot, cells * sizeof(int32_t)));
    PFZ_TRY(pool_alloc(ctx, &s->row_slot, cells * sizeof(uint16_t)));
    PFZ_TRY(pool_alloc(ctx, &s->mag, (size_t)ix->n_blocks * 32 * kSymMag * sizeof(int32_t)));
    PFZ_TRY(pool_alloc(ctx, &s->post_sym, (size_t)ix->piece_cap * kPiece * sizeof(int2)));
    PFZ_TRY(pool_alloc(ctx, &s->keys, (size_t)n * kSymKeep * sizeof(uint64_t)));
    PFZ_TRY(pool_alloc(ctx, &s->push_cnt, (size_t)n * sizeof(int32_t)));
    PFZ_TRY(pool_alloc(ctx, &s->push_buf, (size_t)n * kSymPush * sizeof(uint64_t)));
    PFZ_TRY(pool_alloc(ctx, &s->ovf, (size_t)(n + 1) * sizeof(int32_t)));
    PFZ_TRY(pool_alloc(ctx, &s->part, (size_t)kSymSlicedRows * kSymSlices * kSymKeep * sizeof(uint64_t)));
    for (int q = 0; q + 1 < kSymSides; ++q) {
        PFZ_TRY(pool_alloc(ctx, &s->ovfx[q], (size_t)(n + 1) * sizeof(int32_t)));
        PFZ_TRY(pool_alloc(ctx, &s->partx[q], (size_t)kSymSlicedRows * kSymSlices * kSymKeep * sizeof(uint64_t)));
    }
    PFZ_TRY(pool_alloc(ctx, &s->done, (size_t)(ix->n_blocks + 64) * kSymDoneStride * sizeof(uint32_t)));
    return PFZ_OK;
}

static K3SymState *sym_state_of(pfz_ctx *ctx, const pfz_index *ix)
{
    K3SymState *s = ix->sym;
    if (s) return s->n < 0 ? nullptr : s;
    s = new K3SymState();
    s->ctx = ctx;
    s->n = ix->n_rows;
    ix->sym = s;
    if (getenv("PFZ_K3_SYM_FAIL_ALLOC") || sym_state_alloc(ctx, ix, s) != PFZ_OK) {
        void *const bufs[] = {s->thrv, s->slot4, s->gmin, s->thr_slot, s->row_slot, s->mag, s->post_sym, s->keys, s->push_cnt, s->push_buf, s->ovf, s->part, s->ovfx[0], s->partx[0], s->ovfx[1], s->partx[1], s->ovfx[2], s->partx[2], s->done};
        for (void *p : bufs)
            if (p) pool_free(p);
        *s = K3SymState();
        s->ctx = ctx;
        s->n = -1;
        (void)hipGetLastError();
        return nullptr;
    }
    return s;
}

static int64_t sym_repost_pairs(const pfz_index *ix)
{
    if (ix->pieces_lazy.pending && hipEventQuery(ix->pieces_lazy.ev) == hipSuccess) (void)index_ready(ix);
    (void)hipGetLastError();
    return (ix->pieces_lazy.pending ? ix->piece_cap : (int64_t)ix->n_pieces + 1) * (kPiece / 2);
}

static void sym_fill_args(K3SymArgs &a, const pfz_index *ix, const pfz_csr *A, K3SymState *s, int32_t ntop, int32_t thr0, float scale,
                          float inv_scale)
{
    a.a_indptr = A->indptr;
    a.a_idx = A->indices;
    a.a_val = A->data;
    a.n = (int32_t)ix->n_rows;
    a.tab = ix->tab;
    a.post = ix->post;
    a.post_sym = s->post_sym;
    a.pblk = ix->pblk;
    a.nb = ix->n_blocks;
    a.n_pieces1 = ix->tab + ix->n_cols * ix->n_blocks;
    a.ntop = ntop;
    a.thr0 = thr0;
    a.scale = scale;
    a.inv_scale = inv_scale;
    a.row_begin = 0;
    a.row_end = (int32_t)ix->n_rows;
    a.n_parts = 1;
    a.my_part = 0;
    a.per = (int32_t)ix->n_rows;
    a.thr_by_part = 0;
    a.keys_out = nullptr;
    a.thrv = s->thrv;
    a.slot4 = s->slot4;
    a.gmin = s->gmin;
    a.thr_slot = s->thr_slot;
    a.row_slot = s->row_slot;
    a.mag = s->mag;
    a.n_mag_items = 0;
    a.mag_b0 = 0;
    a.mag_row_end = 0;
    a.keys = s->keys;
    a.push_cnt = s->push_cnt;
    a.push_buf = s->push_buf;
    a.ovf = s->ovf;
    a.part = s->part;
    a.ovf_base = 0;
    a.ovf_max = 0;
    a.n_sl = 1;
    a.out_idx = nullptr;
    a.out_val = nullptr;
    a.done = nullptr;
    a.blk_lo = a.blk_hi = 0;
    a.host_idx = nullptr;
    a.host_val = nullptr;
}

static void sym_launch_pass2(pfz_ctx *ctx, K3SymArgs a, hipStream_t stream = nullptr, int per_cu = 16)
{
    if (!stream) stream = ctx->stream;
    const int nb = a.nb;
    const unsigned grid2 = (unsigned)ctx->prop.multiProcessorCount * (unsigned)per_cu;
    const int per = (nb + kSymSlices - 1) / kSymSlices;
    a.n_mag_items = 0;
    a.n_parts = 1;
    a.n_sl = (nb + per - 1) / per;
    a.ovf_base = 0;
    a.ovf_max = kSymSlicedRows;
    if (a.n_sl > 1) {
        hipLaunchKernelGGL((k3_sym_kernel<kSymC, 2>), dim3(grid2), dim3(64), 0, stream, a);
        hipLaunchKernelGGL(k3_sym_merge_slices, dim3(256), dim3(256), 0, stream, a);
        a.ovf_base = kSymSlicedRows;
    }
    a.n_sl = 1;
    a.ovf_max = a.n;
    hipLaunchKernelGGL((k3_sym_kernel<kSymC, 2>), dim3(grid2), dim3(64), 0, stream, a);
}

int k3_sym_launch(pfz_ctx *ctx, const pfz_index *ix, const pfz_csr *A, int64_t row_begin, int64_t row_end, int32_t ntop,
                  int32_t thr0, float scale, float inv_scale, pfz_topn *out, bool start, bool *declined)
{
    const int64_t n = ix->n_rows;
    const int nb = ix->n_blocks;
    *declined = false;
    K3SymState *s = sym_state_of(ctx, ix);
    if (!s) {
        *declined = true;
        return PFZ_OK;
    }
    s->next_row = -1;
    K3SymArgs a;
    sym_fill_args(a, ix, A, s, ntop, thr0, scale, inv_scale);
    a.out_idx = out->idx;
    a.out_val = out->val;
    if (start) {
        a.row_begin = 0;
        a.row_end = (int32_t)n;
        const unsigned grid0 = (unsigned)std::min<int64_t>(n, (int64_t)ctx->prop.multiProcessorCount * kSymP0PerCu);
        hipLaunchKernelGGL((k3_sym_kernel<kSymC, 0>), dim3(grid0), dim3(64), 0, ctx->stream, a);
        hipLaunchKernelGGL(k3_sym_order, dim3((unsigned)nb), dim3(1024), 0, ctx->stream, a);
        const int64_t pairs = sym_repost_pairs(ix);
        hipLaunchKernelGGL(k3_sym_repost, dim3((unsigned)((pairs + 255) / 256)), dim3(256), 0, ctx->stream, a);
    }
    PFZ_HIP(hipMemsetAsync(s->ovf, 0, sizeof(int32_t), ctx->stream));
    const int64_t last_block_row = (int64_t)(nb - 1) * kSymC;
    a.row_begin = (int32_t)row_begin;
    a.row_end = (int32_t)(row_end < last_block_row ? row_end : last_block_row);
    if (a.row_end < a.row_begin) a.row_end = a.row_begin;
    a.mag_b0 = (int32_t)(row_begin / kSymC);
    a.mag_row_end = (int32_t)row_end;
    a.n_mag_items = (int32_t)(((row_end - 1) / kSymC - a.mag_b0 + 1) * 32 * kSymMag * ((nb - 1 + kSymMagBlocks - 1) / kSymMagBlocks));
#ifdef PFZ_EXPERIMENTS
    if (const char *solo = getenv("PFZ_K3_SYM_SOLO")) {
        int p = 0, np_ = 1;
        if (sscanf(solo, "%d/%d", &p, &np_) == 2 && np_ > 1 && p >= 0 && p < np_ && row_begin == 0) {
            a.n_parts = np_;
            a.my_part = p;
            a.row_begin = p;
        }
    }
    const int rows1 = a.row_end > a.row_begin ? (a.row_end - a.row_begin + a.n_parts - 1) / a.n_parts : 0;
    if (rows1 + a.n_mag_items > 0)
        hipLaunchKernelGGL((k3_sym_kernel<kSymC, 1>), dim3((unsigned)(rows1 + a.n_mag_items)), dim3(64), 0, ctx->stream, a);
    a.n_parts = 1;
    a.my_part = 0;
    if (false)
#endif
    if (a.row_end - a.row_begin + a.n_mag_items > 0)
        hipLaunchKernelGGL((k3_sym_kernel<kSymC, 1>), dim3((unsigned)(a.row_end - a.row_begin + a.n_mag_items)), dim3(64), 0, ctx->stream, a);
    a.n_mag_items = 0;
    a.row_begin = (int32_t)row_begin;
    a.row_end = (int32_t)row_end;
    hipLaunchKernelGGL(k3_sym_merge<4>, dim3((unsigned)((row_end - row_begin + 3) / 4)), dim3(256), 0, ctx->stream, a);
    sym_launch_pass2(ctx, a);
    PFZ_HIP(hipGetLastError());
    s->next_row = row_end;
    s->launches += 1;
    s->rows += row_end - row_begin;
    s->a_serial = A->serial;
    s->out = out;
    s->ntop = ntop;
    s->thr0 = thr0;
    s->scale = scale;
    return PFZ_OK;
}

int k3_sym_launch_streamed(pfz_ctx *ctx, const pfz_index *ix, const pfz_csr *A, int32_t ntop, int32_t thr0, float scale, float inv_scale,
                           pfz_topn *out, int32_t n_ranges, const int64_t *ends, int32_t first_event, int32_t *host_idx, float *host_val,
                           bool *declined)
{
    const int64_t n = ix->n_rows;
    const int nb = ix->n_blocks;
    *declined = false;
    K3SymState *s = sym_state_of(ctx, ix);
    if (!s) {
        *declined = true;
        return PFZ_OK;
    }
    if (!ctx->stream3) {
        int pr_lo = 0, pr_hi = 0;
        PFZ_HIP(hipDeviceGetStreamPriorityRange(&pr_lo, &pr_hi));
        PFZ_HIP(hipStreamCreateWithPriority(&ctx->stream3, hipStreamNonBlocking, pr_hi));
        PFZ_HIP(hipEventCreateWithFlags(&ctx->ev3, hipEventDisableTiming));
        for (int q = 0; q + 1 < kSymSides; ++q) {
            PFZ_HIP(hipStreamCreateWithPriority(&ctx->stream3x[q], hipStreamNonBlocking, pr_hi));
            PFZ_HIP(hipEventCreateWithFlags(&ctx->ev3x[q], hipEventDisableTiming));
        }
    }
    s->next_row = -1;
    K3SymArgs a;
    sym_fill_args(a, ix, A, s, ntop, thr0, scale, inv_scale);
    a.out_idx = out->idx;
    a.out_val = out->val;
    a.host_idx = host_idx;
    a.host_val = host_val;
    a.done = s->done;
    const unsigned grid0 = (unsigned)std::min<int64_t>(n, (int64_t)ctx->prop.multiProcessorCount * kSymP0PerCu);
    hipLaunchKernelGGL((k3_sym_kernel<kSymC, 0>), dim3(grid0), dim3(64), 0, ctx->stream, a);
    hipLaunchKernelGGL(k3_sym_order, dim3((unsigned)nb), dim3(1024), 0, ctx->stream, a);
    const int64_t pairs = sym_repost_pairs(ix);
    hipLaunchKernelGGL(k3_sym_repost, dim3((unsigned)((pairs + 255) / 256)), dim3(256), 0, ctx->stream, a);
    PFZ_HIP(hipEventRecord(ctx->ev3, ctx->stream));
    const int64_t last_block_row = (int64_t)(nb - 1) * kSymC;
    a.row_begin = 0;
    a.row_end = (int32_t)last_block_row;
    a.mag_b0 = 0;
    a.mag_row_end = (int32_t)n;
// ... 49 lines not shown
    s->scale = scale;
    return PFZ_OK;
}

__global__ __launch_bounds__(256) void k3_sym_merge_parts(const uint64_t *__restrict__ keys_all, int32_t n_parts, int32_t n,
                                                           int32_t ntop, float inv_scale, int32_t *__restrict__ out_idx,
                                                           float *__restrict__ out_val)
{
    __shared__ __attribute__((aligned(16))) uint64_t cand_all[4][256];
    const int lane = threadIdx.x & 63, wave = threadIdx.x >> 6;
    const int row = blockIdx.x * 4 + wave;
    if (row >= n) return;
    uint64_t *cand = cand_all[wave];
    TopState st;
    st.cnt = 0;
    st.thr = 0;
    st.pushed = 0;
    const int total = n_parts * ntop;
    for (int e0 = 0; e0 < total; e0 += 64) {
        const int e = e0 + lane;
        const uint64_t k = e < total ? keys_all[((int64_t)(e / ntop) * n + row) * ntop + e % ntop] : 0ull;
        const uint64_t mk = __ballot(k != 0ull);
        if (k) cand[st.cnt + __popcll(mk & ((1ull << lane) - 1ull))] = k;
        st.cnt += __popcll(mk);
    }
    compact<256>(cand, st, ntop, lane);
    for (int q = lane; q < ntop; q += 64) {
        const uint64_t key = q < st.cnt ? cand[q] : 0ull;
        out_idx[(int64_t)row * ntop + q] = key ? (int32_t)(~(uint32_t)key) : -1;
        out_val[(int64_t)row * ntop + q] = key ? (float)(int32_t)(uint32_t)(key >> 32) * inv_scale : 0.f;
    }
}

bool k3_sym_sharded_ok(const pfz_index *ix, const pfz_csr *A, int32_t ntop, int32_t n_parts)
{
    if (A->serial != ix->src_serial || A->n_rows != ix->n_rows) return false;
    if (ix->block_cols != kSymC || !ix->pblk || ntop > kSymKeep || ix->n_blocks < 2 || ix->n_rows >= ((int64_t)1 << 30)) return false;
    if (n_parts < 1 || (int64_t)n_parts * ntop > 256 || n_parts > 64) return false;
    if (ix->sym && ix->sym->n < 0) return false;
    const int force = sym_env_int("PFZ_K3_SYM", -1);
    if (force >= 0) return force != 0;
    return ix->n_rows >= sym_env_int("PFZ_K3_SYM_MIN", 20480) && ix->n_rows <= 250000;
}

static int k3_sym_sharded_body(pfz_ctx *ctx, pfz_comm *comm, const pfz_index *ix, const pfz_csr *A, int32_t ntop, float lower_bound,
                               pfz_topn *out);

int k3_sym_sharded(pfz_ctx *ctx, pfz_comm *comm, const pfz_index *ix, const pfz_csr *A, int32_t ntop, float lower_bound, pfz_topn *out)
{
    const int rc = k3_sym_sharded_body(ctx, comm, ix, A, ntop, lower_bound, out);
    if (rc != PFZ_OK && comm_world(comm) > 1) comm_abort(comm);
    return rc;
}

static int k3_sym_sharded_body(pfz_ctx *ctx, pfz_comm *comm, const pfz_index *ix, const pfz_csr *A, int32_t ntop, float lower_bound,
                               pfz_topn *out)
{
    const int64_t n = ix->n_rows;
    const int nb = ix->n_blocks;
    const int n_parts = comm_world(comm), part = comm_rank(comm);
    K3SymState *s = sym_state_of(ctx, ix);
    if (!s) {
        set_error("pfz_comm_cossim_topn_symmetric: the session buffers of this index could not be allocated");
        return PFZ_ERR_NOMEM;
    }
    float scale, inv_scale;
    int32_t thr0;
    k3_fixed_point(A, ix, lower_bound, &scale, &inv_scale, &thr0);
    s->next_row = -1;
    struct Tmp {
        uint64_t *p = nullptr;
        ~Tmp() { if (p) pool_free(p); }
    } mine, all;
    const size_t list_bytes = (size_t)n * ntop * sizeof(uint64_t);
    PFZ_TRY(pool_alloc(ctx, &mine.p, list_bytes));
    PFZ_TRY(pool_alloc(ctx, &all.p, list_bytes * n_parts));
    K3SymArgs a;
    sym_fill_args(a, ix, A, s, ntop, thr0, scale, inv_scale);
    a.n_parts = n_parts;
    a.my_part = part;
    a.per = (int32_t)((n + n_parts - 1) / n_parts);
    a.thr_by_part = 1;
    a.keys_out = mine.p;
    PFZ_HIP(hipMemsetAsync(s->ovf, 0, sizeof(int32_t), ctx->stream));
    a.row_begin = part;
    a.row_end = (int32_t)n;
    const unsigned mine0 = (unsigned)((n - part + n_parts - 1) / n_parts);
    const unsigned grid0 = std::min<unsigned>(mine0, (unsigned)ctx->prop.multiProcessorCount * (unsigned)kSymP0PerCu);
    if (mine0) hipLaunchKernelGGL((k3_sym_kernel<kSymC, 0>), dim3(grid0), dim3(64), 0, ctx->stream, a);
    PFZ_HIP(hipGetLastError());
    if (n_parts > 1) PFZ_TRY(comm_allgather_bytes(comm, s->thrv + (size_t)part * a.per, s->thrv, (size_t)a.per * sizeof(int32_t)));
    hipLaunchKernelGGL(k3_sym_order, dim3((unsigned)nb), dim3(1024), 0, ctx->stream, a);
    const int64_t pairs = sym_repost_pairs(ix);
    hipLaunchKernelGGL(k3_sym_repost, dim3((unsigned)((pairs + 255) / 256)), dim3(256), 0, ctx->stream, a);
    const int64_t last_block_row = (int64_t)(nb - 1) * kSymC;
    a.row_end = (int32_t)(n < last_block_row ? n : last_block_row);
    const int rows1 = a.row_end > part ? (a.row_end - part + n_parts - 1) / n_parts : 0;
    if (a.row_end < a.row_begin) a.row_end = a.row_begin;
    a.mag_b0 = 0;
    a.mag_row_end = (int32_t)n;
    a.n_mag_items = (int32_t)(nb * 32 * kSymMag * ((nb - 1 + kSymMagBlocks - 1) / kSymMagBlocks));
    hipLaunchKernelGGL((k3_sym_kernel<kSymC, 1>), dim3((unsigned)(rows1 + a.n_mag_items)), dim3(64), 0, ctx->stream, a);
    a.n_mag_items = 0;
    a.row_begin = 0;
    a.row_end = (int32_t)n;
    hipLaunchKernelGGL(k3_sym_merge<4>, dim3((unsigned)((n + 3) / 4)), dim3(256), 0, ctx->stream, a);
    sym_launch_pass2(ctx, a);
    PFZ_HIP(hipGetLastError());
    const uint64_t *lists = mine.p;
    if (n_parts > 1) {
        PFZ_TRY(comm_allgather_bytes(comm, mine.p, all.p, list_bytes));
        lists = all.p;
    }
    hipLaunchKernelGGL(k3_sym_merge_parts, dim3((unsigned)((n + 3) / 4)), dim3(256), 0, ctx->stream, lists, n_parts, (int32_t)n, ntop,
                       inv_scale, out->idx, out->val);
    PFZ_HIP(hipGetLastError());
    s->launches += 1;
    s->rows += n;
    return PFZ_OK;
}

}

extern "C" int pfz_index_symmetric_launches(const pfz_index *ix, int64_t *launches, int64_t *rows)
{
    PFZ_REQUIRE(ix, "pfz_index_symmetric_launches: NULL index");
    if (launches) *launches = ix->sym ? ix->sym->launches : 0;
    if (rows) *rows = ix->sym ? ix->sym->rows : 0;
    return PFZ_OK;
}

extern "C" int pfz_index_symmetric_census(const pfz_index *ix, int64_t *magnet_rows, int64_t *recomputed_rows)
{
    PFZ_REQUIRE(ix, "pfz_index_symmetric_census: NULL index");
    int64_t mags = 0, rec = 0;
    const pfz::K3SymState *s = ix->sym;
    if (s && s->n > 0 && s->launches > 0) {
        PFZ_HIP(hipSetDevice(ix->ctx->device));
        std::vector<int32_t> mag((size_t)ix->n_blocks * 32 * pfz::kSymMag);
        int32_t n_ovf = 0;
        PFZ_TRY(pfz::copy_d2h(ix->ctx, mag.data(), s->mag, mag.size() * sizeof(int32_t)));
        PFZ_TRY(pfz::copy_d2h(ix->ctx, &n_ovf, s->ovf, sizeof(int32_t)));
        for (int32_t r : mag) mags += r >= 0;
        rec = n_ovf;
    }
    if (magnet_rows) *magnet_rows = mags;
    if (recomputed_rows) *recomputed_rows = rec;
    return PFZ_OK;
}

extern "C" int pfz_comm_cossim_topn_symmetric(pfz_comm *c, const pfz_index *ix, const pfz_csr *A, int32_t ntop, float lower_bound,
                                              pfz_topn *out)
{
    PFZ_REQUIRE(c && ix && A && out, "pfz_comm_cossim_topn_symmetric: NULL argument");
    PFZ_REQUIRE(ntop >= 1 && lower_bound == lower_bound, "pfz_comm_cossim_topn_symmetric: ntop must be >= 1 and lower_bound a number");
    PFZ_REQUIRE(out->n_rows >= A->n_rows && out->ntop == ntop, "pfz_comm_cossim_topn_symmetric: result buffer is %lldx%d, need %lldx%d",
                (long long)out->n_rows, out->ntop, (long long)A->n_rows, ntop);
    if (!pfz::k3_sym_sharded_ok(ix, A, ntop, pfz::comm_world(c))) {
        pfz::set_error("pfz_comm_cossim_topn_symmetric: not a job for the symmetric form (the matrix must be the one the index was built "
                       "from, 2048-row blocks, at least two of them, top_n <= 32, ranks x top_n <= 256): ask pfz_index_symmetric_ok first");
        return PFZ_ERR_UNSUPPORTED;
    }
    pfz_ctx *ctx = ix->ctx;
    PFZ_HIP(hipSetDevice(ctx->device));
    pfz::ProfScope ps(ctx, "k3_cossim_topn");
    return pfz::k3_sym_sharded(ctx, c, ix, A, ntop, lower_bound, out);
}
// ... 21 lines not shown
```

### polyfuzz_amd/csrc/pfz_api.hip

```cpp
#include "pfz_internal.h"

#include <stdarg.h>
#include <stdio.h>
#include <stdlib.h>
#include <string.h>

#include <mutex>
#include <unordered_map>

namespace pfz {

static thread_local char g_err[1024] = "";

void set_error(const char *fmt, ...)
{
    va_list ap;
    va_start(ap, fmt);
    vsnprintf(g_err, sizeof(g_err), fmt, ap);
    va_end(ap);
}

int hip_fail(hipError_t e, const char *what, const char *file, int line)
{
    set_error("HIP error %d (%s) in %s at %s:%d", (int)e, hipGetErrorString(e), what, file, line);
    if (e == hipErrorOutOfMemory) return PFZ_ERR_NOMEM;
    if (e == hipErrorNoDevice || e == hipErrorInvalidDevice) return PFZ_ERR_NO_DEVICE;
    return PFZ_ERR_HIP;
}

static std::mutex g_lazy_mu;

int lazy_acquire(pfz_ctx *ctx, LazyI32 *z)
{
    std::lock_guard<std::mutex> lk(g_lazy_mu);
    if (ctx->lazy_slots.empty()) {
        int32_t *chunk = nullptr;
        PFZ_HIP(hipHostMalloc((void **)&chunk, 64 * sizeof(int32_t), hipHostMallocDefault));
        ctx->lazy_chunks.push_back(chunk);
        for (int i = 0; i < 64; ++i) ctx->lazy_slots.push_back(chunk + i);
    }
    if (ctx->lazy_events.empty()) {
        hipEvent_t ev;
        PFZ_HIP(hipEventCreateWithFlags(&ev, hipEventDisableTiming));
        ctx->lazy_events.push_back(ev);
    }
    z->slot = ctx->lazy_slots.back();
    ctx->lazy_slots.pop_back();
    z->ev = ctx->lazy_events.back();
    ctx->lazy_events.pop_back();
    z->pending = false;
    return PFZ_OK;
}

int lazy_mark(pfz_ctx *ctx, LazyI32 *z)
{
    PFZ_HIP(hipEventRecord(z->ev, ctx->stream));
    z->pending = true;
    return PFZ_OK;
}

int lazy_begin(pfz_ctx *ctx, LazyI32 *z, const int32_t *dev)
{
    PFZ_TRY(lazy_acquire(ctx, z));
    PFZ_HIP(hipMemcpyAsync(z->slot, dev, sizeof(int32_t), hipMemcpyDeviceToHost, ctx->stream));
    return lazy_mark(ctx, z);
}

int lazy_get(pfz_ctx *ctx, LazyI32 *z, int32_t *out)
{
    if (z->pending) {
        PFZ_HIP(hipEventSynchronize(z->ev));
        z->value = *z->slot;
        lazy_release(ctx, z);
    }
    *out = z->value;
    return PFZ_OK;
}

void lazy_release(pfz_ctx *ctx, LazyI32 *z)
{
    std::lock_guard<std::mutex> lk(g_lazy_mu);
    if (z->slot) ctx->lazy_slots.push_back(z->slot);
    if (z->ev) ctx->lazy_events.push_back(z->ev);
    z->slot = nullptr;
    z->ev = nullptr;
    z->pending = false;
}

int64_t csr_nnz(const pfz_csr *m)
{
    if (m->nnz_lazy.pending) {
        int32_t v = 0;
        if (lazy_get(m->ctx, &m->nnz_lazy, &v) != PFZ_OK) return -1;
        m->nnz = v;
    }
    return m->nnz;
}

int ensure_scratch(pfz_ctx *ctx, size_t bytes)
{
    if (bytes <= ctx->scratch_bytes) return PFZ_OK;
    if (ctx->scratch) {
        PFZ_HIP(hipStreamSynchronize(ctx->stream));
        PFZ_HIP(hipFree(ctx->scratch));
        ctx->scratch = nullptr;
        ctx->scratch_bytes = 0;
    }
    size_t want = bytes + bytes / 4 + 4096;
    PFZ_HIP(hipMalloc(&ctx->scratch, want));
    ctx->scratch_bytes = want;
    return PFZ_OK;
}

constexpr size_t kStageBytes = (size_t)64 << 20;
constexpr size_t kStageDirect = (size_t)256 << 20;

static int stage_take(pfz_ctx *ctx, size_t bytes, char **out)
{
    if (!ctx->stage) {
        PFZ_HIP(hipHostMalloc((void **)&ctx->stage, kStageBytes, hipHostMallocDefault));
        ctx->stage_bytes = kStageBytes;
        ctx->stage_off = 0;
    }
    const size_t need = (bytes + 255) & ~(size_t)255;
    if (ctx->stage_off + need > ctx->stage_bytes) {
        PFZ_HIP(hipStreamSynchronize(ctx->stream));
        ctx->stage_off = 0;
    }
    *out = ctx->stage + ctx->stage_off;
    ctx->stage_off += need;
    return PFZ_OK;
}

int ensure_side_stream(pfz_ctx *ctx)
{
    if (!ctx->stream2) {
        int pr_lo = 0, pr_hi = 0;
        PFZ_HIP(hipDeviceGetStreamPriorityRange(&pr_lo, &pr_hi));
        PFZ_HIP(hipStreamCreateWithPriority(&ctx->stream2, hipStreamNonBlocking, pr_hi));
        for (hipEvent_t &ev : ctx->side_events) PFZ_HIP(hipEventCreateWithFlags(&ev, hipEventDisableTiming));
    }
    return PFZ_OK;
}

int event_flag_next(pfz_ctx *ctx, int32_t slot, int32_t **flag, int32_t *value)
{
    if (!ctx->evt_flag) {
        PFZ_HIP(hipHostMalloc((void **)&ctx->evt_flag, kEventSlots * sizeof(int32_t), hipHostMallocDefault));
        memset(ctx->evt_flag, 0, kEventSlots * sizeof(int32_t));
    }
    ctx->evt_serial = ctx->evt_serial == 0x7fffffff ? 1 : ctx->evt_serial + 1;
    ctx->evt_want[slot] = ctx->evt_serial;
    *flag = ctx->evt_flag + slot;
    *value = ctx->evt_serial;
    return PFZ_OK;
// ... 90 lines not shown

void pool_free(void *p)
{
    if (!p) return;
    std::lock_guard<std::mutex> lk(g_pool_mu);
    auto it = g_pool_owner.find(p);
    if (it == g_pool_owner.end()) {
        (void)hipFree(p);
        return;
    }
    pfz_ctx *ctx = it->second.first;
    const size_t cls = it->second.second;
    g_pool_owner.erase(it);
    ctx->pool_free_lists[cls].push_back(p);
    ctx->pool_cached_bytes += cls;
    ctx->pool_live_bytes -= cls;
}

int pool_release(pfz_ctx *ctx)
{
    PFZ_HIP(hipSetDevice(ctx->device));
    PFZ_HIP(hipStreamSynchronize(ctx->stream));
    std::lock_guard<std::mutex> lk(g_pool_mu);
    for (auto &kv : ctx->pool_free_lists) {
        for (void *q : kv.second) (void)hipFree(q);
        kv.second.clear();
    }
    ctx->pool_cached_bytes = 0;
    return PFZ_OK;
}

ProfScope::ProfScope(pfz_ctx *c, const char *n, hipStream_t on) : ctx(c), name(n), st(on ? on : c->stream)
{
    if (!ctx->prof) return;
    if (ctx->prof_level == 2 && strncmp(n, "k3_cossim", 9) != 0 && strncmp(n, "k4_indel", 8) != 0 && strncmp(n, "k5_gemm", 7) != 0)
        return;
    auto take = [&]() -> hipEvent_t {
        if (!ctx->event_pool.empty()) {
            hipEvent_t ev = ctx->event_pool.back();
            ctx->event_pool.pop_back();
            return ev;
        }
        hipEvent_t ev = nullptr;
        (void)hipEventCreate(&ev);
        return ev;
    };
    b = take();
    e = take();
    (void)hipEventRecord(b, st);
}

ProfScope::~ProfScope()
{
    static const bool debug_sync = getenv("PFZ_DEBUG_SYNC") != nullptr;
    if (debug_sync) {
        fprintf(stderr, "[pfz] %s ...", name);
        fflush(stderr);
        hipError_t err = hipStreamSynchronize(st);
        fprintf(stderr, " %s\n", hipGetErrorString(err));
    }
    if (!ctx->prof || !b || !e) return;
    (void)hipEventRecord(e, st);
    ProfEntry &pe = ctx->prof_entries[name];
    pe.begin.push_back(b);
    pe.end.push_back(e);
}

static void prof_fold(pfz_ctx *ctx, ProfEntry &pe)
{
    for (size_t i = 0; i < pe.begin.size(); ++i) {
        float ms = 0.f;
        (void)hipEventSynchronize(pe.end[i]);
        if (hipEventElapsedTime(&ms, pe.begin[i], pe.end[i]) == hipSuccess) {
            pe.total_ms += ms;
            pe.launches += 1;
        }
        ctx->event_pool.push_back(pe.begin[i]);
        ctx->event_pool.push_back(pe.end[i]);
    }
    pe.begin.clear();
    pe.end.clear();
}

constexpr int kScanThreads = 256;
constexpr int kScanItems = 16;
constexpr int kScanTile = kScanThreads * kScanItems;

__device__ inline int32_t wave_incl_scan(int32_t v, int lane)
{
#pragma unroll
    for (int d = 1; d < 64; d <<= 1) {
        int32_t o = __shfl_up(v, d, 64);
        if (lane >= d) v += o;
    }
    return v;
}

__device__ inline int32_t block_excl_scan(int32_t v, int32_t *lds4, int32_t *total)
{
    const int lane = threadIdx.x & 63, wave = threadIdx.x >> 6;
    int32_t incl = wave_incl_scan(v, lane);
    if (lane == 63) lds4[wave] = incl;
    __syncthreads();
    int32_t base = 0, tot = 0;
#pragma unroll
    for (int w = 0; w < kScanThreads / 64; ++w) {
        int32_t s = lds4[w];
        if (w < wave) base += s;
        tot += s;
    }
    __syncthreads();
    *total = tot;
    return base + incl - v;
}

__global__ __launch_bounds__(kScanThreads) void k_scan_tile_sums(const int32_t *__restrict__ in, int64_t n,
                                                                 int32_t *__restrict__ tile_sums)
{
    __shared__ int32_t lds4[kScanThreads / 64];
    const int64_t base = (int64_t)blockIdx.x * kScanTile + (int64_t)threadIdx.x * kScanItems;
    int32_t s = 0;
#pragma unroll
    for (int i = 0; i < kScanItems; ++i) {
        int64_t p = base + i;
        if (p < n) s += in[p];
    }
    int32_t tot;
    (void)block_excl_scan(s, lds4, &tot);
    if (threadIdx.x == 0) tile_sums[blockIdx.x] = tot;
}

__global__ __launch_bounds__(kScanThreads) void k_scan_sums(int32_t *__restrict__ tile_sums, int64_t n_tiles,
                                                            int32_t *__restrict__ grand_total)
{
    __shared__ int32_t lds4[kScanThreads / 64];
    int32_t carry = 0;
    for (int64_t t0 = 0; t0 < n_tiles; t0 += kScanThreads) {
        int64_t p = t0 + threadIdx.x;
        int32_t v = (p < n_tiles) ? tile_sums[p] : 0;
        int32_t tot;
        int32_t ex = block_excl_scan(v, lds4, &tot);
        if (p < n_tiles) tile_sums[p] = carry + ex;
        carry += tot;
    }
    if (threadIdx.x == 0) *grand_total = carry;
}

__global__ __launch_bounds__(kScanThreads) void k_scan_apply(int32_t *__restrict__ data, int64_t n,
                                                             const int32_t *__restrict__ tile_sums)
{
    __shared__ int32_t lds4[kScanThreads / 64];
    const int64_t base = (int64_t)blockIdx.x * kScanTile + (int64_t)threadIdx.x * kScanItems;
    int32_t v[kScanItems];
    int32_t s = 0;
#pragma unroll
    for (int i = 0; i < kScanItems; ++i) {
        int64_t p = base + i;
        v[i] = (p < n) ? data[p] : 0;
        s += v[i];
    }
    int32_t tot;
    int32_t ex = block_excl_scan(s, lds4, &tot) + tile_sums[blockIdx.x];
#pragma unroll
    for (int i = 0; i < kScanItems; ++i) {
        int64_t p = base + i;
        if (p < n) data[p] = ex;
        ex += v[i];
    }
}

__global__ __launch_bounds__(kScanThreads) void k_scan_lookback(int32_t *__restrict__ data, int64_t n, uint64_t *__restrict__ state,
                                                                uint32_t *__restrict__ ticket, uint32_t epoch4, int32_t n_tiles,
                                                                int32_t *__restrict__ host_total)
{
    __shared__ int32_t lds4[kScanThreads / 64];
    __shared__ int32_t s_tile, s_prefix;
    if (threadIdx.x == 0) s_tile = (int32_t)atomicAdd(ticket, 1u);
    __syncthreads();
    const int tile = s_tile;
    const int64_t base = (int64_t)tile * kScanTile + (int64_t)threadIdx.x * kScanItems;
    int32_t v[kScanItems];
    int32_t s = 0;
#pragma unroll
    for (int i = 0; i < kScanItems; ++i) {
        const int64_t p = base + i;
        v[i] = (p < n) ? data[p] : 0;
        s += v[i];
    }
    int32_t tot;
    int32_t ex = block_excl_scan(s, lds4, &tot);
    if (threadIdx.x == 0) {
        int32_t prefix = 0;
        if (tile > 0) {
            __hip_atomic_store(&state[tile], ((uint64_t)(epoch4 + 1u) << 32) | (uint32_t)tot, __ATOMIC_RELAXED, __HIP_MEMORY_SCOPE_AGENT);
            for (int p = tile - 1;; --p) {
                uint64_t w;
                for (;;) {
                    w = __hip_atomic_load(&state[p], __ATOMIC_RELAXED, __HIP_MEMORY_SCOPE_AGENT);
                    const uint32_t f = (uint32_t)(w >> 32);
                    if (f == epoch4 + 1u || f == epoch4 + 2u) break;
                    __builtin_amdgcn_s_sleep(2);
                }
                prefix += (int32_t)(uint32_t)w;
                if ((uint32_t)(w >> 32) == epoch4 + 2u) break;
            }
        }
        __hip_atomic_store(&state[tile], ((uint64_t)(epoch4 + 2u) << 32) | (uint32_t)(prefix + tot), __ATOMIC_RELAXED,
                           __HIP_MEMORY_SCOPE_AGENT);
        s_prefix = prefix;
        if (tile == n_tiles - 1) {
            data[n] = prefix + tot;
            if (host_total) __hip_atomic_store(host_total, prefix + tot, __ATOMIC_RELAXED, __HIP_MEMORY_SCOPE_SYSTEM);
            *ticket = 0u;
        }
    }
    __syncthreads();
    ex += s_prefix;
#pragma unroll
    for (int i = 0; i < kScanItems; ++i) {
        const int64_t p = base + i;
        if (p < n) data[p] = ex;
        ex += v[i];
    }
}

int exclusive_scan_i32(pfz_ctx *ctx, int32_t *data, int64_t n, LazyI32 *total)
{
    if (n <= 0) {
        PFZ_HIP(hipMemsetAsync(data, 0, sizeof(int32_t), ctx->stream));
        return total ? lazy_begin(ctx, total, data) : PFZ_OK;
    }
    const int64_t n_tiles = (n + kScanTile - 1) / kScanTile;
    static const bool three = getenv("PFZ_SCAN3") != nullptr;
    if (!three && n_tiles < (1 << 24)) {
        if ((size_t)n_tiles > ctx->scan_tiles) {
            size_t cap = ctx->scan_tiles ? ctx->scan_tiles : 1024;
            while (cap < (size_t)n_tiles) cap *= 2;
            uint64_t *fresh = nullptr;
            PFZ_TRY(pool_alloc(ctx, &fresh, (cap + 1) * sizeof(uint64_t)));
            PFZ_HIP(hipMemsetAsync(fresh, 0, (cap + 1) * sizeof(uint64_t), ctx->stream));
            if (ctx->scan_state) pool_free(ctx->scan_state);
            ctx->scan_state = fresh;
            ctx->scan_tiles = cap;
            ctx->scan_epoch = 0;
        }
        if (ctx->scan_epoch >= (1u << 29)) {
            PFZ_HIP(hipMemsetAsync(ctx->scan_state, 0, (ctx->scan_tiles + 1) * sizeof(uint64_t), ctx->stream));
            ctx->scan_epoch = 0;
        }
        const uint32_t epoch4 = ++ctx->scan_epoch * 4u;
        if (total) PFZ_TRY(lazy_acquire(ctx, total));
        hipLaunchKernelGGL(k_scan_lookback, dim3((unsigned)n_tiles), dim3(kScanThreads), 0, ctx->stream, data, n, ctx->scan_state,
                           (uint32_t *)(ctx->scan_state + ctx->scan_tiles), epoch4, (int32_t)n_tiles, total ? total->slot : nullptr);
        PFZ_HIP(hipGetLastError());
        return total ? lazy_mark(ctx, total) : PFZ_OK;
    }
    PFZ_TRY(ensure_scratch(ctx, (size_t)n_tiles * sizeof(int32_t)));
    int32_t *tile_sums = (int32_t *)ctx->scratch;
    hipLaunchKernelGGL(k_scan_tile_sums, dim3((unsigned)n_tiles), dim3(kScanThreads), 0, ctx->stream, data, n, tile_sums);
    hipLaunchKernelGGL(k_scan_sums, dim3(1), dim3(kScanThreads), 0, ctx->stream, tile_sums, n_tiles, data + n);
    hipLaunchKernelGGL(k_scan_apply, dim3((unsigned)n_tiles), dim3(kScanThreads), 0, ctx->stream, data, n, tile_sums);
    PFZ_HIP(hipGetLastError());
    return total ? lazy_begin(ctx, total, data + n) : PFZ_OK;
}

}

using namespace pfz;

extern "C" {

int pfz_version(void) { return PFZ_VERSION; }

const char *pfz_last_error(void) { return pfz::g_err; }

int pfz_device_count(void)
{
    int n = 0;
    if (hipGetDeviceCount(&n) != hipSuccess) return 0;
    return n;
}

int pfz_ctx_create(int device, pfz_ctx **out)
{
    PFZ_REQUIRE(out != nullptr, "pfz_ctx_create: out is NULL");
    *out = nullptr;
    int n = 0;
    hipError_t e = hipGetDeviceCount(&n);
    if (e != hipSuccess || n <= 0) {
        set_error("pfz_ctx_create: no HIP device visible (hipGetDeviceCount -> %d, %s); "
                  "libpolyfuzz_hip has no CPU fallback", (int)e, hipGetErrorString(e));
        return PFZ_ERR_NO_DEVICE;
    }
    PFZ_REQUIRE(device >= 0 && device < n, "pfz_ctx_create: device %d out of range [0,%d)", device, n);
    PFZ_HIP(hipSetDevice(device));
    pfz_ctx *ctx = new pfz_ctx();
    ctx->device = device;
    PFZ_HIP(hipGetDeviceProperties(&ctx->prop, device));
    if (strncmp(ctx->prop.gcnArchName, "gfx950", 6) != 0) {
        set_error("pfz_ctx_create: device %d is %s; this library ships gfx950 code objects only",
                  device, ctx->prop.gcnArchName);
        delete ctx;
        return PFZ_ERR_NO_DEVICE;
    }
    PFZ_HIP(hipStreamCreateWithFlags(&ctx->stream, hipStreamNonBlocking));
    for (int i = 0; i < kEventSlots; ++i) PFZ_HIP(hipEventCreate(&ctx->events[i]));
    *out = ctx;
    return PFZ_OK;
}

void pfz_ctx_destroy(pfz_ctx *ctx)
{
    if (!ctx) return;
    (void)hipSetDevice(ctx->device);
    (void)hipStreamSynchronize(ctx->stream);
    for (auto &kv : ctx->prof_entries) prof_fold(ctx, kv.second);
    for (hipEvent_t ev : ctx->event_pool) (void)hipEventDestroy(ev);
    for (hipEvent_t ev : ctx->lazy_events) (void)hipEventDestroy(ev);
    for (int32_t *c : ctx->lazy_chunks) (void)hipHostFree(c);
    for (int i = 0; i < kEventSlots; ++i)
        if (ctx->events[i]) (void)hipEventDestroy(ctx->events[i]);
    if (ctx->scratch) (void)hipFree(ctx->scratch);
    if (ctx->stage) (void)hipHostFree(ctx->stage);
    if (ctx->stage2) (void)hipHostFree(ctx->stage2);
    if (ctx->evt_flag) (void)hipHostFree(ctx->evt_flag);
    if (ctx->mirror) (void)hipHostFree(ctx->mirror);
    for (char *p : ctx->rows_stage)
        if (p) (void)hipHostFree(p);
    for (hipEvent_t ev : ctx->rows_ev)
        if (ev) (void)hipEventDestroy(ev);
    for (hipEvent_t ev : ctx->side_events)
        if (ev) (void)hipEventDestroy(ev);
    if (ctx->stream2) {
        (void)hipStreamSynchronize(ctx->stream2);
        (void)hipStreamDestroy(ctx->stream2);
    }
    if (ctx->stream3) {
        (void)hipStreamSynchronize(ctx->stream3);
        (void)hipStreamDestroy(ctx->stream3);
    }
    if (ctx->ev3) (void)hipEventDestroy(ctx->ev3);
    for (int q = 0; q < 3; ++q) {
        if (ctx->stream3x[q]) {
            (void)hipStreamSynchronize(ctx->stream3x[q]);
// ... 142 lines not shown
    }
    PFZ_REQUIRE(nnz == 0 || (indices && data), "pfz_csr_upload: NULL indices/data");
    PFZ_HIP(hipSetDevice(ctx->device));
    Owner<pfz_csr, pfz_csr_free> m(new pfz_csr());
    m->ctx = ctx;
    m->n_rows = n_rows;
    m->n_cols = n_cols;
    m->nnz = nnz;
    m->nnz_cap = nnz;
    std::vector<int32_t> ip32((size_t)n_rows + 1);
    for (int64_t i = 0; i <= n_rows; ++i) {
        if (i > 0 && indptr[i] < indptr[i - 1]) {
            set_error("pfz_csr_upload: indptr not monotone at row %lld", (long long)i);
            return PFZ_ERR_INVALID;
        }
        ip32[(size_t)i] = (int32_t)indptr[i];
    }
    {
        double mx = 0.0;
        for (int64_t i = 0; i < n_rows; ++i) {
            double ss = 0.0;
            for (int64_t p = indptr[i]; p < indptr[i + 1]; ++p) {
                if (indices[p] < 0 || indices[p] >= n_cols) {
                    set_error("pfz_csr_upload: row %lld has column index %d outside [0, %lld)", (long long)i,
                              indices[p], (long long)n_cols);
                    return PFZ_ERR_INVALID;
                }
                ss += (double)data[p] * (double)data[p];
            }
            if (!(ss == ss) || ss > 1e60) {
                set_error("pfz_csr_upload: row %lld has a non-finite or huge norm", (long long)i);
                return PFZ_ERR_INVALID;
            }
            if (ss > mx) mx = ss;
        }
        m->max_norm = (float)(sqrt(mx) * 1.000001);
    }
    PFZ_TRY(pool_alloc(ctx, &m->indptr, (size_t)(n_rows + 1) * sizeof(int32_t)));
    PFZ_TRY(pool_alloc(ctx, &m->indices, (size_t)(nnz > 0 ? nnz : 1) * sizeof(int32_t)));
    PFZ_TRY(pool_alloc(ctx, &m->data, (size_t)(nnz > 0 ? nnz : 1) * sizeof(float)));
    PFZ_TRY(copy_h2d(ctx, m->indptr, ip32.data(), (size_t)(n_rows + 1) * sizeof(int32_t)));
    if (nnz > 0) {
        PFZ_TRY(copy_h2d(ctx, m->indices, indices, (size_t)nnz * sizeof(int32_t)));
        PFZ_TRY(copy_h2d(ctx, m->data, data, (size_t)nnz * sizeof(float)));
    }
    *out = m.release();
    return PFZ_OK;
}

int pfz_csr_shape(const pfz_csr *m, int64_t *n_rows, int64_t *n_cols, int64_t *nnz)
{
    PFZ_REQUIRE(m, "pfz_csr_shape: NULL matrix");
    if (n_rows) *n_rows = m->n_rows;
    if (n_cols) *n_cols = m->n_cols;
    if (nnz) {
        *nnz = csr_nnz(m);
        if (*nnz < 0) return PFZ_ERR_HIP;
    }
    return PFZ_OK;
}

int pfz_csr_download(pfz_ctx *ctx, const pfz_csr *m, int64_t *indptr, int32_t *indices, float *data)
{
    PFZ_REQUIRE(ctx && m, "pfz_csr_download: NULL argument");
    PFZ_HIP(hipSetDevice(ctx->device));
    PFZ_HIP(hipStreamSynchronize(ctx->stream));
    if (indptr) {
        std::vector<int32_t> ip32((size_t)m->n_rows + 1);
        PFZ_TRY(copy_d2h(ctx, ip32.data(), m->indptr, ip32.size() * sizeof(int32_t)));
        for (size_t i = 0; i < ip32.size(); ++i) indptr[i] = ip32[i];
    }
    const int64_t nnz = csr_nnz(m);
    if (nnz < 0) return PFZ_ERR_HIP;
    if (indices && nnz > 0) PFZ_TRY(copy_d2h(ctx, indices, m->indices, (size_t)nnz * sizeof(int32_t)));
    if (data && nnz > 0) PFZ_TRY(copy_d2h(ctx, data, m->data, (size_t)nnz * sizeof(float)));
    return PFZ_OK;
}

void pfz_csr_free(pfz_csr *m)
{
    if (!m) return;
    if (m->ctx) (void)hipSetDevice(m->ctx->device);
    if (m->nnz_lazy.pending || m->nnz_lazy.slot) {
        if (m->nnz_lazy.ev) (void)hipEventSynchronize(m->nnz_lazy.ev);
        pfz::lazy_release(m->ctx, &m->nnz_lazy);
    }
    if (m->indptr) pool_free(m->indptr);
    if (m->indices) pool_free(m->indices);
    if (m->data) pool_free(m->data);
    delete m;
}


int pfz_topn_alloc(pfz_ctx *ctx, int64_t n_rows, int32_t ntop, pfz_topn **out)
{
    PFZ_REQUIRE(ctx && out && n_rows >= 0 && ntop >= 1, "pfz_topn_alloc: bad args");
    PFZ_HIP(hipSetDevice(ctx->device));
    Owner<pfz_topn, pfz_topn_free> t(new pfz_topn());
    t->ctx = ctx;
    t->n_rows = n_rows;
    t->ntop = ntop;
    size_t n = (size_t)(n_rows > 0 ? n_rows : 1) * (size_t)ntop;
    const size_t idx_bytes = (n * sizeof(int32_t) + 255) & ~(size_t)255;
    PFZ_TRY(pool_alloc(ctx, &t->idx, idx_bytes + n * sizeof(float)));
    t->val = (float *)((char *)t->idx + idx_bytes);
    *out = t.release();
    return PFZ_OK;
}

void pfz_topn_free(pfz_topn *t)
{
    if (!t) return;
    if (t->ctx) (void)hipSetDevice(t->ctx->device);
    if (t->idx) pool_free(t->idx);
    delete t;
}

int pfz_topn_clear(pfz_ctx *ctx, pfz_topn *t)
{
    PFZ_REQUIRE(ctx && t, "pfz_topn_clear: NULL argument");
    PFZ_HIP(hipSetDevice(ctx->device));
    const size_t n = (size_t)t->n_rows * (size_t)t->ntop;
    if (n == 0) return PFZ_OK;
    PFZ_HIP(hipMemsetAsync(t->idx, 0xFF, n * sizeof(int32_t), ctx->stream));
    PFZ_HIP(hipMemsetAsync(t->val, 0, n * sizeof(float), ctx->stream));
    return PFZ_OK;
}

int pfz_topn_download(pfz_ctx *ctx, const pfz_topn *t, int32_t *out_idx, float *out_val)
{
    PFZ_REQUIRE(ctx && t, "pfz_topn_download: NULL argument");
    PFZ_HIP(hipSetDevice(ctx->device));
    size_t n = (size_t)t->n_rows * (size_t)t->ntop;
    if (n == 0) {
        PFZ_HIP(hipStreamSynchronize(ctx->stream));
        return PFZ_OK;
    }
    const size_t span = (size_t)((const char *)t->val - (const char *)t->idx) + n * sizeof(float);
    if (out_idx && out_val && span <= (64u << 10)) {
        char *st = nullptr;
        PFZ_TRY(stage_take(ctx, span, &st));
        PFZ_HIP(hipMemcpyAsync(st, t->idx, span, hipMemcpyDeviceToHost, ctx->stream));
        PFZ_HIP(hipStreamSynchronize(ctx->stream));
        memcpy(out_idx, st, n * sizeof(int32_t));
        memcpy(out_val, st + ((const char *)t->val - (const char *)t->idx), n * sizeof(float));
        ctx->stage_off = 0;
        return PFZ_OK;
    }
    if (out_idx) PFZ_TRY(copy_d2h(ctx, out_idx, t->idx, n * sizeof(int32_t)));
    if (out_val) PFZ_TRY(copy_d2h(ctx, out_val, t->val, n * sizeof(float)));
    return PFZ_OK;
}

int pfz_topn_download_rows_after(pfz_ctx *ctx, const pfz_topn *t, int64_t row_begin, int64_t row_end, int32_t event_slot,
                                 int32_t *out_idx, float *out_val)
{
    PFZ_REQUIRE(ctx && t && out_idx && out_val, "pfz_topn_download_rows_after: NULL argument");
    PFZ_REQUIRE(row_begin >= 0 && row_begin <= row_end && row_end <= t->n_rows, "pfz_topn_download_rows_after: bad row range");
    PFZ_REQUIRE(event_slot >= 0 && event_slot < kEventSlots, "pfz_topn_download_rows_after: bad event slot %d", event_slot);
    PFZ_HIP(hipSetDevice(ctx->device));
    const size_t n = (size_t)(row_end - row_begin) * (size_t)t->ntop;
    if (n == 0) return PFZ_OK;
    PFZ_TRY(ensure_side_stream(ctx));
    const size_t bytes = n * (sizeof(int32_t) + sizeof(float));
    if (bytes > ctx->stage2_bytes) {
        PFZ_HIP(hipStreamSynchronize(ctx->stream2));
        if (ctx->stage2) PFZ_HIP(hipHostFree(ctx->stage2));
// ... 106 lines not shown
```

### polyfuzz_amd/csrc/pfz_internal.h

```cpp
#pragma once

#include <hip/hip_runtime.h>
#include <stdint.h>
#include <string>
#include <vector>
#include <map>
#include <atomic>

#include "polyfuzz_hip.h"

namespace pfz {

void set_error(const char *fmt, ...) __attribute__((format(printf, 1, 2)));
int hip_fail(hipError_t e, const char *what, const char *file, int line);

#define PFZ_HIP(call)                                                      \
    do {                                                                   \
        hipError_t _e = (call);                                            \
        if (_e != hipSuccess) return pfz::hip_fail(_e, #call, __FILE__, __LINE__); \
    } while (0)

#define PFZ_TRY(call)                 \
    do {                              \
        int _s = (call);              \
        if (_s != PFZ_OK) return _s;  \
    } while (0)

#define PFZ_REQUIRE(cond, ...)                    \
    do {                                          \
        if (!(cond)) {                            \
            pfz::set_error(__VA_ARGS__);          \
            return PFZ_ERR_INVALID;               \
        }                                         \
    } while (0)

constexpr int kWave = 64;
constexpr int kHistWords = 36864;
constexpr int kEventSlots = 64;

inline uint64_t next_serial()
{
    static std::atomic<uint64_t> s{1};
    return s.fetch_add(1);
}
struct K3SymState;

struct LazyI32 {
    hipEvent_t ev = nullptr;
    int32_t *slot = nullptr;
    bool pending = false;
    int32_t value = 0;
};

struct ProfEntry {
    std::vector<hipEvent_t> begin, end;
    double total_ms = 0.0;
    int64_t launches = 0;
};

}

struct pfz_ctx {
    int device = -1;
    hipStream_t stream = nullptr;
    hipStream_t stream2 = nullptr;
    hipEvent_t side_events[4] = {};
    hipStream_t stream3 = nullptr;
    hipEvent_t ev3 = nullptr;
    hipStream_t stream3x[3] = {nullptr, nullptr, nullptr};
    hipEvent_t ev3x[3] = {nullptr, nullptr, nullptr};
    hipDeviceProp_t prop;
    hipEvent_t events[pfz::kEventSlots] = {};
    bool prof = false;
    int prof_level = 0;
    std::map<std::string, pfz::ProfEntry> prof_entries;
    std::vector<hipEvent_t> event_pool;
    void *scratch = nullptr;
    size_t scratch_bytes = 0;
    char *stage = nullptr;
    size_t stage_bytes = 0, stage_off = 0;
    char *stage2 = nullptr;
    size_t stage2_bytes = 0;
    int32_t *evt_flag = nullptr;
    int32_t evt_want[pfz::kEventSlots] = {};
    int32_t evt_serial = 0;
    struct RowsJob { const pfz_topn *t = nullptr; int64_t row_begin = 0, row_end = 0; int32_t slot = -1; bool issued = false; } rows_job[2];
    char *mirror = nullptr;
    size_t mirror_bytes = 0;
    char *rows_stage[2] = {};
    size_t rows_bytes[2] = {}, rows_n[2] = {};
    hipEvent_t rows_ev[2] = {};
    uint64_t *scan_state = nullptr;
    size_t scan_tiles = 0;
    uint32_t scan_epoch = 0;
    std::vector<int32_t *> lazy_slots;
    std::vector<hipEvent_t> lazy_events;
    std::vector<int32_t *> lazy_chunks;
    std::map<size_t, std::vector<void *>> pool_free_lists;
    size_t pool_cached_bytes = 0, pool_live_bytes = 0;
};

struct pfz_csr {
    pfz_ctx *ctx = nullptr;
    int64_t n_rows = 0, n_cols = 0;
    mutable int64_t nnz = 0;
    mutable pfz::LazyI32 nnz_lazy;
    int64_t nnz_cap = 0;
    int32_t *indptr = nullptr;
    int32_t *indices = nullptr;
    float *data = nullptr;
    float max_norm = 1.f;
    uint64_t serial = pfz::next_serial();
};

struct pfz_index {
    pfz_ctx *ctx = nullptr;
    int64_t n_rows = 0, n_cols = 0;
    int32_t block_cols = 0, n_blocks = 0;
    mutable int32_t n_pieces = 0;
    mutable int64_t nnz = 0;
    mutable pfz::LazyI32 pieces_lazy, nnz_lazy;
    int64_t piece_cap = 0;
    int32_t *tab_base = nullptr;
    int32_t *tab = nullptr;
    int2 *post = nullptr;
    uint16_t *pblk = nullptr;
    float max_norm = 1.f;
    uint64_t src_serial = 0;
    mutable pfz::K3SymState *sym = nullptr;
};

struct pfz_topn {
    pfz_ctx *ctx = nullptr;
    int64_t n_rows = 0;
    int32_t ntop = 0;
    int32_t *idx = nullptr;
    float *val = nullptr;
};

struct pfz_strings {
    pfz_ctx *ctx = nullptr;
    int64_t n = 0, n_units = 0;
    int32_t char_width = 1;
    void *chars = nullptr;
    bool chars_in_offsets = false;
    int64_t *offsets = nullptr;
    int64_t max_len = 0;
    std::vector<int64_t> h_off;
    struct pfz_indel_plan *indel_plan = nullptr;
    struct pfz_fuzz_forms *fuzz_forms = nullptr;
    struct pfz_fuzz_plan *fuzz_plan = nullptr;
    uint64_t cache_gen = 0;
    uint64_t *slots = nullptr;
    size_t slots_cap = 0;
    int32_t *row_cnt = nullptr;
};

void pfz_indel_plan_free(struct pfz_indel_plan *p);
void pfz_fuzz_forms_free(struct pfz_fuzz_forms *f);
void pfz_fuzz_plan_free(struct pfz_fuzz_plan *p);

struct pfz_tfidf {
    pfz_ctx *ctx = nullptr;
    pfz_tfidf_params params;
    uint64_t gen = 0;
    int32_t bits_per_char = 0;
    int32_t code_bits = 0;
    uint32_t *alpha_map = nullptr;
    int64_t alpha_map_len = 0;
    std::vector<uint32_t> alphabet;
    uint32_t *bitmap = nullptr;
    int32_t *prefix = nullptr;
    int64_t n_groups = 0;
    int64_t vocab = 0, n_docs = 0;
    uint64_t *vcodes = nullptr;
    int32_t *df = nullptr;
    double *idf = nullptr;
};

namespace pfz {

inline int decode_skip_codes(std::vector<int32_t> &v)
{
    bool eq = false, le = false;
    for (int32_t x : v) {
        eq |= x >= 0;
        le |= x <= -2;
    }
    if (eq && le) return -1;
    if (!le) return 0;
    for (int32_t &x : v) x = x <= -2 ? -2 - x : -1;
    return 1;
}
__host__ __device__ inline bool choice_left_out(int orig, int s, int up_to) { return up_to ? orig <= s : orig == s; }

template <typename T, void (*Free)(T *)> struct Owner {
    T *p;
    explicit Owner(T *q) : p(q) {}
    ~Owner() { if (p) Free(p); }
    Owner(const Owner &) = delete;
    Owner &operator=(const Owner &) = delete;
    T *operator->() const { return p; }
    T *release() { T *q = p; p = nullptr; return q; }
};

int ensure_scratch(pfz_ctx *ctx, size_t bytes);
int lazy_begin(pfz_ctx *ctx, LazyI32 *z, const int32_t *dev);
int lazy_acquire(pfz_ctx *ctx, LazyI32 *z);
int lazy_mark(pfz_ctx *ctx, LazyI32 *z);
int lazy_get(pfz_ctx *ctx, LazyI32 *z, int32_t *out);
void lazy_release(pfz_ctx *ctx, LazyI32 *z);
int64_t csr_nnz(const pfz_csr *m);
int index_ready(const pfz_index *ix);
int ensure_side_stream(pfz_ctx *ctx);
int event_flag_next(pfz_ctx *ctx, int32_t slot, int32_t **flag, int32_t *value);
int copy_h2d(pfz_ctx *ctx, void *dst_dev, const void *src_host, size_t bytes);
int copy_d2h(pfz_ctx *ctx, void *dst_host, const void *src_dev, size_t bytes);
struct ProfScope {
    pfz_ctx *ctx;
    const char *name;
    hipStream_t st;
    hipEvent_t b = nullptr, e = nullptr;
    ProfScope(pfz_ctx *c, const char *n, hipStream_t on = nullptr);
    ~ProfScope();
};

int pool_alloc_raw(pfz_ctx *ctx, void **p, size_t bytes);
template <typename T> inline int pool_alloc(pfz_ctx *ctx, T **p, size_t bytes)
{
    return pool_alloc_raw(ctx, (void **)p, bytes);
}
void pool_free(void *p);
int pool_release(pfz_ctx *ctx);

int comm_rank(const pfz_comm *c);
int comm_world(const pfz_comm *c);
int comm_allgather_bytes(pfz_comm *c, const void *send, void *recv, size_t bytes_per_rank);
int comm_allreduce_sum_i32(pfz_comm *c, int32_t *buf, size_t n);
int comm_allreduce_sum_i64(pfz_comm *c, int64_t *buf, size_t n);
int comm_agree(pfz_comm *c, bool mine, bool *all);
void comm_abort(pfz_comm *c);

int exclusive_scan_i32(pfz_ctx *ctx, int32_t *data, int64_t n, LazyI32 *total = nullptr);

int best_to_topn(pfz_ctx *ctx, const int32_t *d_idx, const double *d_score, int64_t n, pfz_topn *out);

int64_t sort_codes_capacity(int64_t n);
int sort_codes_u64(pfz_ctx *ctx, const uint64_t *in, uint64_t *out, int64_t n);

}
```

Measured before the change: 3602 billion.

## Fuse long-row tiles into short-row launch and scan directly from source arrays

Long-row processing is folded into the short-row vectorize kernel as extra workgroups when every row fits in LDS. The separate copy-then-scan steps for row counts are replaced by a scan that reads from a source pointer. The index-pieces computation is fused with the lookback scan through a shared scan header, and the pad and head work is merged. The aim is to cut kernel launches and extra memory passes during TF-IDF build and index construction, at the cost of more complex kernels, larger LDS use in the combined launch, and a changed layout for the heavy-list counter.

```diff
diff --git a/polyfuzz_amd/csrc/k1_vectorize.hip b/polyfuzz_amd/csrc/k1_vectorize.hip
--- a/polyfuzz_amd/csrc/k1_vectorize.hip
+++ b/polyfuzz_amd/csrc/k1_vectorize.hip
@@ -609,32 +609,6 @@
     }
 }
 
-__global__ __launch_bounds__(256) void k_rows_short(const int64_t *__restrict__ off, int64_t n, int32_t R,
-                                                     VocabView V, uint64_t *__restrict__ slots,
-                                                     const int32_t *__restrict__ row_cnt,
-                                                     int32_t *__restrict__ row_nnz, DfSink df, ListB B = ListB{})
-{
-    const int lane = threadIdx.x & 63;
-    unsigned bx = blockIdx.x;
-    if (bx >= B.grid0) {
-        bx -= B.grid0;
-        off = B.off;
-        n = B.n;
-        slots = B.slots;
-        row_cnt = B.row_cnt;
-        row_nnz = B.row_cnt + (B.n + 1);
-    }
-    const int64_t row = (int64_t)bx * 4 + (threadIdx.x >> 6);
-    if (row >= n) return;
-    const int cnt = row_cnt[row];
-    if (cnt > kShortMax) return;
-    if (cnt == 0) {
-        if (lane == 0) row_nnz[row] = 0;
-        return;
-    }
-    rows_short_row(V, slots + off[row] * R, cnt, lane, row_nnz + row, row, df);
-}
-
 template <typename KEYS>
 __device__ inline void rows_long_body(KEYS keys, int cnt, const VocabView &V, uint64_t *base, int32_t *row_nnz_out,
                                       DfSink df, int *sh_heads, int *sh_valid)
@@ -696,17 +670,16 @@
     }
 }
 
-__global__ __launch_bounds__(256) void k_rows_long(const int64_t *__restrict__ off, int64_t n, int32_t R, VocabView V,
-                                                    uint64_t *__restrict__ slots,
-                                                    const int32_t *__restrict__ row_cnt,
-                                                    int32_t *__restrict__ row_nnz, DfSink df,
-                                                    uint32_t *__restrict__ giant_scratch, int64_t giant_stride)
+__device__ inline void rows_long_tiles(unsigned wg, unsigned n_wg, const int64_t *__restrict__ off, int64_t n, int32_t R,
+                                       const VocabView &V, uint64_t *__restrict__ slots, const int32_t *__restrict__ row_cnt,
+                                       int32_t *__restrict__ row_nnz, DfSink df, uint32_t *__restrict__ giant_scratch,
+                                       int64_t giant_stride)
 {
     __shared__ uint32_t lds_keys[kLongMax];
     __shared__ int sh_heads, sh_valid, n_long;
     __shared__ int long_rows[kLongTile];
     const int64_t n_tiles = (n + kLongTile - 1) / kLongTile;
-    for (int64_t tile = blockIdx.x; tile < n_tiles; tile += gridDim.x) {
+    for (int64_t tile = wg; tile < n_tiles; tile += n_wg) {
         if (threadIdx.x == 0) n_long = 0;
         __syncthreads();
         const int64_t mine = tile * kLongTile + threadIdx.x;
@@ -720,12 +693,53 @@
             if (cnt <= kLongMax)
                 rows_long_body(&lds_keys[0], cnt, V, base, row_nnz + row, df, &sh_heads, &sh_valid);
             else
-                rows_long_body(giant_scratch + (int64_t)blockIdx.x * giant_stride, cnt, V, base, row_nnz + row, df,
+                rows_long_body(giant_scratch + (int64_t)wg * giant_stride, cnt, V, base, row_nnz + row, df,
                                &sh_heads, &sh_valid);
             __syncthreads();
         }
         __syncthreads();
     }
+}
+
+__global__ __launch_bounds__(256) void k_rows_long(const int64_t *__restrict__ off, int64_t n, int32_t R, VocabView V,
+                                                    uint64_t *__restrict__ slots,
+                                                    const int32_t *__restrict__ row_cnt,
+                                                    int32_t *__restrict__ row_nnz, DfSink df,
+                                                    uint32_t *__restrict__ giant_scratch, int64_t giant_stride)
+{
+    rows_long_tiles(blockIdx.x, gridDim.x, off, n, R, V, slots, row_cnt, row_nnz, df, giant_scratch, giant_stride);
+}
+
+__global__ __launch_bounds__(256) void k_rows_short(const int64_t *__restrict__ off, int64_t n, int32_t R,
+                                                     VocabView V, uint64_t *__restrict__ slots,
+                                                     const int32_t *__restrict__ row_cnt,
+                                                     int32_t *__restrict__ row_nnz, DfSink df, ListB B = ListB{},
+                                                     unsigned long_grid = 0)
+{
+    const int lane = threadIdx.x & 63;
+    unsigned bx = blockIdx.x;
+    if (bx < long_grid) {
+        rows_long_tiles(bx, long_grid, off, n, R, V, slots, row_cnt, row_nnz, df, nullptr, 0);
+        return;
+    }
+    bx -= long_grid;
+    if (bx >= B.grid0) {
+        bx -= B.grid0;
+        off = B.off;
+        n = B.n;
+        slots = B.slots;
+        row_cnt = B.row_cnt;
+        row_nnz = B.row_cnt + (B.n + 1);
+    }
+    const int64_t row = (int64_t)bx * 4 + (threadIdx.x >> 6);
+    if (row >= n) return;
+    const int cnt = row_cnt[row];
+    if (cnt > kShortMax) return;
+    if (cnt == 0) {
+        if (lane == 0) row_nnz[row] = 0;
+        return;
+    }
+    rows_short_row(V, slots + off[row] * R, cnt, lane, row_nnz + row, row, df);
 }
 
 __global__ __launch_bounds__(256) void k_idf(const int32_t *__restrict__ df, int64_t vocab, double n_docs,
@@ -803,12 +817,6 @@
         indices[o + t] = (int32_t)e.x;
         data[o + t] = (float)v;
     }
-}
-
-__global__ __launch_bounds__(256) void k_copy_i32(const int32_t *__restrict__ src, int64_t n, int32_t *__restrict__ dst)
-{
-    const int64_t i = (int64_t)blockIdx.x * 256 + threadIdx.x;
-    if (i < n) dst[i] = src[i];
 }
 
 static inline unsigned grid_for(int64_t n, int per_block = 256) { return (unsigned)((n + per_block - 1) / per_block); }
@@ -921,6 +929,8 @@
     const int R = v->params.ngram_hi - v->params.ngram_lo + 1;
     VocabView V{v->bitmap, v->prefix, v->vcodes, v->vocab};
     int32_t *row_nnz = s->row_cnt + (s->n + 1);
+    const int64_t max_cnt = s->max_len * R;
+    bool long_done = max_cnt <= kShortMax;
     if (!short_done) {
         ListB B;
         unsigned grid_b = 0;
@@ -932,12 +942,16 @@
             B.grid0 = grid_for(s->n, 4);
             grid_b = grid_for(sb->n, 4);
         }
+        unsigned long_grid = 0;
+        if (!long_done && max_cnt <= kLongMax) {
+            long_grid = (unsigned)std::min<int64_t>((s->n + kLongTile - 1) / kLongTile, 2048);
+            long_done = true;
+        }
         ProfScope ps(ctx, "k2_rows_short");
-        hipLaunchKernelGGL(k_rows_short, dim3(grid_for(s->n, 4) + grid_b), dim3(256), 0, ctx->stream, s->offsets, s->n, R, V,
-                           s->slots, s->row_cnt, row_nnz, df, B);
-    }
-    if (s->max_len * R > kShortMax) {
-        const int64_t max_cnt = s->max_len * R;
+        hipLaunchKernelGGL(k_rows_short, dim3(grid_for(s->n, 4) + grid_b + long_grid), dim3(256), 0, ctx->stream, s->offsets, s->n, R, V,
+                           s->slots, s->row_cnt, row_nnz, df, B, long_grid);
+    }
+    if (!long_done) {
         const int64_t n_tiles = (s->n + kLongTile - 1) / kLongTile;
         unsigned grid = (unsigned)std::min<int64_t>(n_tiles, 2048);
         uint32_t *giant = nullptr;
@@ -995,8 +1009,7 @@
         pfz_strings *s = lists[li];
         if (!s || s->n == 0) continue;
         PFZ_TRY(pool_alloc(ctx, &code_off[li].p, (size_t)(s->n + 1) * sizeof(int32_t)));
-        hipLaunchKernelGGL(k_copy_i32, dim3(grid_for(s->n)), dim3(256), 0, ctx->stream, s->row_cnt, s->n, (int32_t *)code_off[li].p);
-        PFZ_TRY(exclusive_scan_i32(ctx, (int32_t *)code_off[li].p, s->n));
+        PFZ_TRY(exclusive_scan_i32(ctx, (int32_t *)code_off[li].p, s->n, nullptr, s->row_cnt));
         int32_t t = 0;
         PFZ_HIP(hipMemcpyAsync(&t, (int32_t *)code_off[li].p + s->n, sizeof(int32_t), hipMemcpyDeviceToHost, ctx->stream));
         PFZ_HIP(hipStreamSynchronize(ctx->stream));
@@ -1487,8 +1500,7 @@
             }
             PFZ_TRY(lazy_mark(ctx, &m->nnz_lazy));
         } else {
-            hipLaunchKernelGGL(k_copy_i32, dim3(grid_for(s->n)), dim3(256), 0, ctx->stream, row_nnz, s->n, m->indptr);
-            PFZ_TRY(exclusive_scan_i32(ctx, m->indptr, s->n, &m->nnz_lazy));
+            PFZ_TRY(exclusive_scan_i32(ctx, m->indptr, s->n, &m->nnz_lazy, row_nnz));
             ProfScope ps(ctx, "k2_finalize");
             hipLaunchKernelGGL(k_finalize<false>, dim3(grid_for(s->n, 16)), dim3(256), 0, ctx->stream, s->offsets, s->n, R, s->slots,
                                m->indptr, v->idf, m->indices, m->data, nullptr, nullptr);
diff --git a/polyfuzz_amd/csrc/k3_cossim_topn.hip b/polyfuzz_amd/csrc/k3_cossim_topn.hip
--- a/polyfuzz_amd/csrc/k3_cossim_topn.hip
+++ b/polyfuzz_amd/csrc/k3_cossim_topn.hip
@@ -1,4 +1,5 @@
 #include "k3_core.h"
+#include "pfz_scan.h"
 
 #include <algorithm>
 #include <math.h>
@@ -41,48 +42,95 @@
 }
 
 constexpr int kSub = 4;
-__global__ __launch_bounds__(256) void k_index_pieces(int32_t *__restrict__ cnt, int32_t *__restrict__ sub, int64_t slots,
-                                                       int32_t *__restrict__ tab, int32_t *__restrict__ heavy, int32_t heavy_cap,
-                                                       int32_t bank_min)
-{
-    const int64_t i = (int64_t)blockIdx.x * 256 + threadIdx.x;
-    int c = 0;
-    if (i == 0) tab[-1] = 1;
-    if (i < slots) {
-        if (sub) {
-            int4 v = ((const int4 *)sub)[i];
-            c = v.x + v.y + v.z + v.w;
-            if (c) ((int4 *)sub)[i] = make_int4(0, v.x, v.x + v.y, v.x + v.y + v.z);
-            cnt[i] = c;
-        } else {
-            c = cnt[i];
-        }
-        tab[i] = (c + kPiece - 1) / kPiece;
-    } else if (i < slots + 2) {
-        tab[i] = 0;
-    }
-    const bool h = heavy && i < slots && c >= bank_min;
+__device__ inline int index_pieces_of(int64_t i, int4 v, int32_t *__restrict__ cnt, int32_t *__restrict__ sub, int64_t slots,
+                                      int32_t *__restrict__ heavy_n, int32_t *__restrict__ heavy, int32_t heavy_cap, int32_t bank_min)
+{
+    const int c = v.x + v.y + v.z + v.w;
+    if (sub && i >= 0 && i < slots) {
+        if (c) ((int4 *)sub)[i] = make_int4(0, v.x, v.x + v.y, v.x + v.y + v.z);
+        cnt[i] = c;
+    }
+    const bool h = heavy && c >= bank_min;
     const uint64_t m = __ballot(h);
     if (m) {
         const int lane = threadIdx.x & 63, first = __ffsll((long long)m) - 1;
         int base = 0;
-        if (lane == first) base = atomicAdd(&heavy[0], __popcll(m));
+        if (lane == first) base = atomicAdd(heavy_n, __popcll(m));
         base = __shfl(base, first, 64);
         const int at = base + __popcll(m & ((1ull << lane) - 1ull));
-        if (h && at < heavy_cap) heavy[1 + at] = (int32_t)i;
-    }
-}
-
-__global__ __launch_bounds__(256) void k_index_pad(const int32_t *__restrict__ cnt, const int32_t *__restrict__ tab,
-                                                    int64_t slots, int2 *__restrict__ post,
-                                                    uint16_t *__restrict__ pblk, int32_t nb, const int32_t *__restrict__ nnz_dev,
-                                                    int32_t *__restrict__ nnz_host)
+        if (h && at < heavy_cap) heavy[at] = (int32_t)i;
+    }
+    return (c + kPiece - 1) / kPiece;
+}
+
+__global__ __launch_bounds__(256) void k_index_pieces(int32_t *__restrict__ cnt, int32_t *__restrict__ sub, int64_t slots,
+                                                       int32_t *__restrict__ tab, int32_t *__restrict__ heavy_n,
+                                                       int32_t *__restrict__ heavy, int32_t heavy_cap, int32_t bank_min)
 {
     const int64_t i = (int64_t)blockIdx.x * 256 + threadIdx.x;
-    if (i == 0) __hip_atomic_store(nnz_host, *nnz_dev, __ATOMIC_RELAXED, __HIP_MEMORY_SCOPE_SYSTEM);
-    if (i < kPiece) post[i] = make_int2((int)i * 4, 0);
-    if (i == 0 && pblk) pblk[0] = 0;
-    if (i >= slots) return;
+    if (i == 0) tab[-1] = 1;
+    int4 v = make_int4(0, 0, 0, 0);
+    if (i < slots) v = sub ? ((const int4 *)sub)[i] : make_int4(cnt[i], 0, 0, 0);
+    const int pieces = index_pieces_of(i, v, cnt, sub, slots, heavy_n, heavy, heavy_cap, bank_min);
+    if (i < slots + 2) tab[i] = pieces;
+}
+
+__global__ __launch_bounds__(kScanThreads) void k_index_pieces_scan(int32_t *__restrict__ cnt, int32_t *__restrict__ sub, int64_t slots,
+                                                                    int32_t *__restrict__ tab_base, int32_t *__restrict__ heavy_n,
+                                                                    int32_t *__restrict__ heavy, int32_t heavy_cap, int32_t bank_min,
+                                                                    ScanPass pass, int32_t *__restrict__ host_total)
+{
+    __shared__ int32_t lds4[kScanThreads / 64];
+    __shared__ int32_t s_tile, s_prefix;
+    __shared__ __attribute__((aligned(16))) int32_t s_pieces[kScanTile];
+    __shared__ int32_t s_heavy[kScanTile];
+    __shared__ int s_heavy_n, s_heavy_base;
+    const int tile = scan_take_tile(pass.ticket, &s_tile);
+    const int64_t p0 = (int64_t)tile * kScanTile + threadIdx.x;
+    int4 c4[kScanItems];
+#pragma unroll
+    for (int k = 0; k < kScanItems; ++k) {
+        const int64_t i = p0 + k * kScanThreads - 1;
+        c4[k] = make_int4(0, 0, 0, 0);
+        if (i >= 0 && i < slots) c4[k] = sub ? ((const int4 *)sub)[i] : make_int4(cnt[i], 0, 0, 0);
+    }
+    if (threadIdx.x == 0) s_heavy_n = 0;
+    __syncthreads();
+#pragma unroll
+    for (int k = 0; k < kScanItems; ++k) {
+        const int64_t p = p0 + k * kScanThreads;
+        const int c = c4[k].x + c4[k].y + c4[k].z + c4[k].w;
+        if (sub && p >= 1 && p <= slots) {
+            if (c) ((int4 *)sub)[p - 1] = make_int4(0, c4[k].x, c4[k].x + c4[k].y, c4[k].x + c4[k].y + c4[k].z);
+            cnt[p - 1] = c;
+        }
+        if (heavy && c >= bank_min) s_heavy[atomicAdd(&s_heavy_n, 1)] = (int32_t)(p - 1);
+        s_pieces[threadIdx.x + k * kScanThreads] = p == 0 ? 1 : (c + kPiece - 1) / kPiece;
+    }
+    __syncthreads();
+    if (s_heavy_n > 0) {
+        if (threadIdx.x == 0) s_heavy_base = atomicAdd(heavy_n, s_heavy_n);
+        __syncthreads();
+        for (int t = threadIdx.x; t < s_heavy_n; t += kScanThreads)
+            if (s_heavy_base + t < heavy_cap) heavy[s_heavy_base + t] = s_heavy[t];
+    }
+    __syncthreads();
+    int32_t v[kScanItems];
+#pragma unroll
+    for (int i = 0; i < kScanItems; i += 4) {
+        const int4 q = ((const int4 *)s_pieces)[(threadIdx.x * kScanItems + i) / 4];
+        v[i] = q.x;
+        v[i + 1] = q.y;
+        v[i + 2] = q.z;
+        v[i + 3] = q.w;
+    }
+    if (scan_lookback_tile(v, tile, tab_base, slots + 1, pass.state, pass.ticket, pass.epoch4, pass.n_tiles, host_total, lds4, &s_prefix))
+        tab_base[slots + 2] = 0;
+}
+
+__device__ inline void index_pad_list(int64_t i, const int32_t *__restrict__ cnt, const int32_t *__restrict__ tab,
+                                      int2 *__restrict__ post, uint16_t *__restrict__ pblk, int32_t nb)
+{
     const int c = cnt[i];
     if (c == 0) return;
     if (pblk) {
@@ -94,6 +142,24 @@
     const int64_t base = (int64_t)tab[i] * kPiece;
     const int end = (c + kPiece - 1) & ~(kPiece - 1);
     for (int p = c; p < end; ++p) post[base + p] = make_int2(((((int)i & 3) << 4) | (p & 15)) * 4, 0);
+}
+
+__device__ inline void index_pad_head(int t, int2 *__restrict__ post, uint16_t *__restrict__ pblk,
+                                      const int32_t *__restrict__ nnz_dev, int32_t *__restrict__ nnz_host)
+{
+    if (t == 0) __hip_atomic_store(nnz_host, *nnz_dev, __ATOMIC_RELAXED, __HIP_MEMORY_SCOPE_SYSTEM);
+    if (t < kPiece) post[t] = make_int2(t * 4, 0);
+    if (t == 0 && pblk) pblk[0] = 0;
+}
+
+__global__ __launch_bounds__(256) void k_index_pad(const int32_t *__restrict__ cnt, const int32_t *__restrict__ tab,
+                                                    int64_t slots, int2 *__restrict__ post,
+                                                    uint16_t *__restrict__ pblk, int32_t nb, const int32_t *__restrict__ nnz_dev,
+                                                    int32_t *__restrict__ nnz_host)
+{
+    const int64_t i = (int64_t)blockIdx.x * 256 + threadIdx.x;
+    if (blockIdx.x == 0) index_pad_head((int)threadIdx.x, post, pblk, nnz_dev, nnz_host);
+    if (i < slots) index_pad_list(i, cnt, tab, post, pblk, nb);
 }
 
 __global__ __launch_bounds__(1024) void k_index_count_lds(const int32_t *__restrict__ indptr,
@@ -148,11 +214,19 @@
                                                           int32_t block, int32_t words,
                                                           const int32_t *__restrict__ tab ,
                                                           const int32_t *__restrict__ sub_first ,
-                                                          int2 *__restrict__ post)
+                                                          int2 *__restrict__ post, const int32_t *__restrict__ cnt, int64_t slots,
+                                                          uint16_t *__restrict__ pblk, const int32_t *__restrict__ nnz_dev,
+                                                          int32_t *__restrict__ nnz_host)
 {
     __shared__ uint32_t h[kHistWords];
     for (int t = threadIdx.x; t < words; t += 1024) h[t] = 0u;
     __syncthreads();
+    if (threadIdx.x >= 512) {
+        const int64_t per_wg = (slots + gridDim.x - 1) / gridDim.x;
+        const int64_t i0 = (int64_t)blockIdx.x * per_wg, i1 = i0 + per_wg < slots ? i0 + per_wg : slots;
+        for (int64_t i = i0 + (threadIdx.x - 512); i < i1; i += 512) index_pad_list(i, cnt, tab, post, pblk, nb);
+        if (blockIdx.x == 0) index_pad_head((int)threadIdx.x - 512, post, pblk, nnz_dev, nnz_host);
+    }
     const int b = blockIdx.x / kSub, q = blockIdx.x % kSub;
     const int per = block / kSub;
     const int blk0 = b * block;
@@ -316,6 +390,7 @@
 
 constexpr int kBankMin = 64, kBankCap = 1024;
 __global__ __launch_bounds__(256) void k_index_bank_order(const int32_t *__restrict__ cnt, const int32_t *__restrict__ tab,
+                                                           const int32_t *__restrict__ heavy_n,
                                                            const int32_t *__restrict__ heavy, int32_t heavy_cap,
                                                            int2 *__restrict__ post)
 {
@@ -324,11 +399,11 @@
     const int lane = threadIdx.x & 63, wave = threadIdx.x >> 6;
     int2 *buf = s_buf[wave];
     int *bc = s_cnt[wave];
-    const int n_heavy = min(heavy[0], heavy_cap);
+    const int n_heavy = min(*heavy_n, heavy_cap);
     const int n_waves = (int)gridDim.x * 4;
     for (int h = (int)blockIdx.x * 4 + wave; h < n_heavy; h += n_waves) {
         {
-            const int64_t slot = heavy[1 + h];
+            const int64_t slot = heavy[h];
             const int c = min(cnt[slot], kBankCap);
             const int64_t base = (int64_t)tab[slot] * kPiece;
             if (lane < 32) bc[lane] = 0;
@@ -460,9 +535,12 @@
     PFZ_TRY(pool_alloc(ctx, &ix->tab_base, (size_t)(slots + 3) * sizeof(int32_t)));
     ix->tab = ix->tab_base + 1;
     PFZ_TRY(pool_alloc(ctx, &cnt.p, (size_t)(slots + 2) * sizeof(int32_t)));
+    int32_t *heavy_n = nullptr;
     if (lds_hist && any) {
-        PFZ_TRY(pool_alloc(ctx, &sub.p, (size_t)(slots + 1) * kSub * sizeof(int32_t)));
-        PFZ_HIP(hipMemsetAsync(sub.p, 0, (size_t)slots * kSub * sizeof(int32_t), ctx->stream));
+        const size_t sub_words = (size_t)(slots + 1) * kSub;
+        PFZ_TRY(pool_alloc(ctx, &sub.p, (sub_words + 4) * sizeof(int32_t)));
+        heavy_n = sub.p + sub_words;
+        PFZ_HIP(hipMemsetAsync(sub.p, 0, (sub_words + 4) * sizeof(int32_t), ctx->stream));
     } else {
         PFZ_HIP(hipMemsetAsync(cnt.p, 0, (size_t)(slots + 2) * sizeof(int32_t), ctx->stream));
     }
@@ -472,13 +550,13 @@
     const int32_t bank_min = kBankMin;
     const int32_t heavy_cap = (int32_t)std::min<int64_t>(slots, (int64_t)1 << 22);
     Tmp heavy;
-    if (bank_order) {
-        PFZ_TRY(pool_alloc(ctx, &heavy.p, (size_t)(heavy_cap + 1) * sizeof(int32_t)));
-        PFZ_HIP(hipMemsetAsync(heavy.p, 0, sizeof(int32_t), ctx->stream));
-    }
+    if (bank_order) PFZ_TRY(pool_alloc(ctx, &heavy.p, (size_t)heavy_cap * sizeof(int32_t)));
     const int32_t words = (int32_t)((B->n_cols + 1) / 2);
     const unsigned row_grid = (unsigned)((B->n_rows * 16 + 255) / 256);
     const unsigned slot_grid = (unsigned)((slots + kPiece + 255) / 256);
+    ScanPass pass;
+    bool single = false;
+    PFZ_TRY(scan_single_pass(ctx, slots + 1, &pass, &single));
     {
         ProfScope ps(ctx, "k_index_count");
         if (any && lds_hist)
@@ -487,10 +565,18 @@
         else if (any)
             hipLaunchKernelGGL(k_index_count, dim3(row_grid), dim3(256), 0, ctx->stream, B->indptr, B->indices,
                                (int32_t)B->n_rows, (int32_t)nb, block, cnt.p);
-        hipLaunchKernelGGL(k_index_pieces, dim3(slot_grid), dim3(256), 0, ctx->stream, cnt.p, lds_hist && any ? sub.p : nullptr, slots,
-                           ix->tab, heavy.p, heavy_cap, bank_min);
-    }
-    PFZ_TRY(exclusive_scan_i32(ctx, ix->tab_base, slots + 1, &ix->pieces_lazy));
+        if (single) {
+            PFZ_TRY(lazy_acquire(ctx, &ix->pieces_lazy));
+            hipLaunchKernelGGL(k_index_pieces_scan, dim3((unsigned)pass.n_tiles), dim3(kScanThreads), 0, ctx->stream, cnt.p,
+                               lds_hist && any ? sub.p : nullptr, slots, ix->tab_base, heavy_n, bank_order ? heavy.p : nullptr, heavy_cap,
+                               bank_min, pass, ix->pieces_lazy.slot);
+            PFZ_TRY(lazy_mark(ctx, &ix->pieces_lazy));
+        } else {
+            hipLaunchKernelGGL(k_index_pieces, dim3(slot_grid), dim3(256), 0, ctx->stream, cnt.p, lds_hist && any ? sub.p : nullptr, slots,
+                               ix->tab, heavy_n, bank_order ? heavy.p : nullptr, heavy_cap, bank_min);
+        }
+    }
+    if (!single) PFZ_TRY(exclusive_scan_i32(ctx, ix->tab_base, slots + 1, &ix->pieces_lazy));
     const int64_t nnz_bound = B->nnz_lazy.pending ? B->nnz_cap : B->nnz;
     int64_t piece_cap = nnz_bound / kPiece + std::min<int64_t>(slots, nnz_bound) + 1;
     if (piece_cap > kPieceBoundMax) {
@@ -511,20 +597,23 @@
         PFZ_TRY(pool_alloc(ctx, &ix->pblk, (size_t)piece_cap * sizeof(uint16_t)));
     {
         ProfScope ps(ctx, "k_index_fill");
-        hipLaunchKernelGGL(k_index_pad, dim3(slot_grid), dim3(256), 0, ctx->stream, cnt.p, ix->tab, slots, ix->post, ix->pblk, (int32_t)nb,
-                           B->indptr + B->n_rows, ix->nnz_lazy.slot);
+        if (any && lds_hist) {
+            hipLaunchKernelGGL(k_index_fill_lds, dim3((unsigned)nb * kSub), dim3(1024), 0, ctx->stream, B->indptr, B->indices,
+                               B->data, (int32_t)B->n_rows, (int32_t)nb, block, words, ix->tab, sub.p, ix->post, cnt.p, slots, ix->pblk,
+                               B->indptr + B->n_rows, ix->nnz_lazy.slot);
+        } else {
+            hipLaunchKernelGGL(k_index_pad, dim3(slot_grid), dim3(256), 0, ctx->stream, cnt.p, ix->tab, slots, ix->post, ix->pblk, (int32_t)nb,
+                               B->indptr + B->n_rows, ix->nnz_lazy.slot);
+            if (any)
+                hipLaunchKernelGGL(k_index_fill, dim3(row_grid), dim3(256), 0, ctx->stream, B->indptr, B->indices, B->data,
+                                   (int32_t)B->n_rows, (int32_t)nb, block, cnt.p, ix->tab, ix->post);
+        }
         PFZ_TRY(lazy_mark(ctx, &ix->nnz_lazy));
-        if (any && lds_hist)
-            hipLaunchKernelGGL(k_index_fill_lds, dim3((unsigned)nb * kSub), dim3(1024), 0, ctx->stream, B->indptr, B->indices,
-                               B->data, (int32_t)B->n_rows, (int32_t)nb, block, words, ix->tab, sub.p, ix->post);
-        else if (any)
-            hipLaunchKernelGGL(k_index_fill, dim3(row_grid), dim3(256), 0, ctx->stream, B->indptr, B->indices, B->data,
-                               (int32_t)B->n_rows, (int32_t)nb, block, cnt.p, ix->tab, ix->post);
     }
     if (bank_order) {
         ProfScope ps(ctx, "k_index_bank_order");
         hipLaunchKernelGGL(k_index_bank_order, dim3((unsigned)ctx->prop.multiProcessorCount * 4), dim3(256), 0, ctx->stream, cnt.p,
-                           ix->tab, heavy.p, heavy_cap, ix->post);
+                           ix->tab, heavy_n, heavy.p, heavy_cap, ix->post);
     }
     PFZ_HIP(hipGetLastError());
     *out = ix.release();
@@ -538,7 +627,7 @@
     k3_sym_free(ix);
     for (LazyI32 *z : {&ix->pieces_lazy, &ix->nnz_lazy})
         if (z->pending || z->slot) {
-            if (z->ev) (void)hipEventSynchronize(z->ev);
+            (void)lazy_wait(ix->ctx, z);
             lazy_release(ix->ctx, z);
         }
     if (ix->tab_base) pool_free(ix->tab_base);
diff --git a/polyfuzz_amd/csrc/k3_symmetric.hip b/polyfuzz_amd/csrc/k3_symmetric.hip
--- a/polyfuzz_amd/csrc/k3_symmetric.hip
+++ b/polyfuzz_amd/csrc/k3_symmetric.hip
@@ -92,6 +92,7 @@
     const int b = blockIdx.x, lane = threadIdx.x & 63, wave = threadIdx.x >> 6;
     if (threadIdx.x < 256) s_gmin[threadIdx.x] = kNoThr;
     if (threadIdx.x == 0 && a.done) a.done[b * kSymDoneStride] = 0u;
+    if (threadIdx.x == 0 && b == 0) a.ovf[0] = 0;
     __syncthreads();
     for (int rho = wave * 2; rho < wave * 2 + 2; ++rho) {
         const int r = rho + 32 * lane;
@@ -738,8 +739,7 @@
 
 static int64_t sym_repost_pairs(const pfz_index *ix)
 {
-    if (ix->pieces_lazy.pending && hipEventQuery(ix->pieces_lazy.ev) == hipSuccess) (void)index_ready(ix);
-    (void)hipGetLastError();
+    if (ix->pieces_lazy.pending && lazy_ready(&ix->pieces_lazy)) (void)index_ready(ix);
     return (ix->pieces_lazy.pending ? ix->piece_cap : (int64_t)ix->n_pieces + 1) * (kPiece / 2);
 }
 
@@ -838,7 +838,7 @@
         const int64_t pairs = sym_repost_pairs(ix);
         hipLaunchKernelGGL(k3_sym_repost, dim3((unsigned)((pairs + 255) / 256)), dim3(256), 0, ctx->stream, a);
     }
-    PFZ_HIP(hipMemsetAsync(s->ovf, 0, sizeof(int32_t), ctx->stream));
+    if (!start) PFZ_HIP(hipMemsetAsync(s->ovf, 0, sizeof(int32_t), ctx->stream));
     const int64_t last_block_row = (int64_t)(nb - 1) * kSymC;
     a.row_begin = (int32_t)row_begin;
     a.row_end = (int32_t)(row_end < last_block_row ? row_end : last_block_row);
@@ -1054,7 +1054,6 @@
     a.per = (int32_t)((n + n_parts - 1) / n_parts);
     a.thr_by_part = 1;
     a.keys_out = mine.p;
-    PFZ_HIP(hipMemsetAsync(s->ovf, 0, sizeof(int32_t), ctx->stream));
     a.row_begin = part;
     a.row_end = (int32_t)n;
     const unsigned mine0 = (unsigned)((n - part + n_parts - 1) / n_parts);
diff --git a/polyfuzz_amd/csrc/pfz_api.hip b/polyfuzz_amd/csrc/pfz_api.hip
--- a/polyfuzz_amd/csrc/pfz_api.hip
+++ b/polyfuzz_amd/csrc/pfz_api.hip
@@ -1,10 +1,12 @@
 #include "pfz_internal.h"
+#include "pfz_scan.h"
 
 #include <stdarg.h>
 #include <stdio.h>
 #include <stdlib.h>
 #include <string.h>
 
+#include <chrono>
 #include <mutex>
 #include <unordered_map>
 
@@ -39,38 +41,82 @@
         ctx->lazy_chunks.push_back(chunk);
         for (int i = 0; i < 64; ++i) ctx->lazy_slots.push_back(chunk + i);
     }
-    if (ctx->lazy_events.empty()) {
-        hipEvent_t ev;
-        PFZ_HIP(hipEventCreateWithFlags(&ev, hipEventDisableTiming));
-        ctx->lazy_events.push_back(ev);
-    }
     z->slot = ctx->lazy_slots.back();
     ctx->lazy_slots.pop_back();
-    z->ev = ctx->lazy_events.back();
-    ctx->lazy_events.pop_back();
+    __atomic_store_n(z->slot, kLazyUnset, __ATOMIC_RELEASE);
+    z->ev = nullptr;
     z->pending = false;
     return PFZ_OK;
 }
 
-int lazy_mark(pfz_ctx *ctx, LazyI32 *z)
-{
+int lazy_mark(pfz_ctx *, LazyI32 *z)
+{
+    z->pending = true;
+    return PFZ_OK;
+}
+
+int lazy_begin(pfz_ctx *ctx, LazyI32 *z, const int32_t *dev)
+{
+    PFZ_TRY(lazy_acquire(ctx, z));
+    {
+        std::lock_guard<std::mutex> lk(g_lazy_mu);
+        if (ctx->lazy_events.empty()) {
+            hipEvent_t ev;
+            PFZ_HIP(hipEventCreateWithFlags(&ev, hipEventDisableTiming));
+            ctx->lazy_events.push_back(ev);
+        }
+        z->ev = ctx->lazy_events.back();
+        ctx->lazy_events.pop_back();
+    }
+    PFZ_HIP(hipMemcpyAsync(z->slot, dev, sizeof(int32_t), hipMemcpyDeviceToHost, ctx->stream));
     PFZ_HIP(hipEventRecord(z->ev, ctx->stream));
     z->pending = true;
     return PFZ_OK;
 }
 
-int lazy_begin(pfz_ctx *ctx, LazyI32 *z, const int32_t *dev)
-{
-    PFZ_TRY(lazy_acquire(ctx, z));
-    PFZ_HIP(hipMemcpyAsync(z->slot, dev, sizeof(int32_t), hipMemcpyDeviceToHost, ctx->stream));
-    return lazy_mark(ctx, z);
+bool lazy_ready(const LazyI32 *z)
+{
+    if (!z->pending) return true;
+    if (z->ev) {
+        const bool fired = hipEventQuery(z->ev) == hipSuccess;
+        (void)hipGetLastError();
+        return fired;
+    }
+    return __atomic_load_n(z->slot, __ATOMIC_ACQUIRE) != kLazyUnset;
+}
+
+int lazy_wait(pfz_ctx *ctx, const LazyI32 *z)
+{
+    if (!z->pending) return PFZ_OK;
+    if (z->ev) {
+        PFZ_HIP(hipEventSynchronize(z->ev));
+        return PFZ_OK;
+    }
+    auto t0 = std::chrono::steady_clock::now();
+    while (__atomic_load_n(z->slot, __ATOMIC_ACQUIRE) == kLazyUnset) {
+        __builtin_ia32_pause();
+        const auto t1 = std::chrono::steady_clock::now();
+        if (t1 - t0 < std::chrono::seconds(1)) continue;
+        t0 = t1;
+        const hipError_t e = hipStreamQuery(ctx->stream);
+        if (e == hipErrorNotReady) {
+            (void)hipGetLastError();
+            continue;
+        }
+        PFZ_HIP(e);
+        if (__atomic_load_n(z->slot, __ATOMIC_ACQUIRE) == kLazyUnset) {
+            set_error("a value the device owes the host was never written (stream idle)");
+            return PFZ_ERR_HIP;
+        }
+    }
+    return PFZ_OK;
 }
 
 int lazy_get(pfz_ctx *ctx, LazyI32 *z, int32_t *out)
 {
     if (z->pending) {
-        PFZ_HIP(hipEventSynchronize(z->ev));
-        z->value = *z->slot;
+        PFZ_TRY(lazy_wait(ctx, z));
+        z->value = __atomic_load_n(z->slot, __ATOMIC_ACQUIRE);
         lazy_release(ctx, z);
     }
     *out = z->value;
@@ -327,38 +373,6 @@
     pe.end.clear();
 }
 
-constexpr int kScanThreads = 256;
-constexpr int kScanItems = 16;
-constexpr int kScanTile = kScanThreads * kScanItems;
-
-__device__ inline int32_t wave_incl_scan(int32_t v, int lane)
-{
-#pragma unroll
-    for (int d = 1; d < 64; d <<= 1) {
-        int32_t o = __shfl_up(v, d, 64);
-        if (lane >= d) v += o;
-    }
-    return v;
-}
-
-__device__ inline int32_t block_excl_scan(int32_t v, int32_t *lds4, int32_t *total)
-{
-    const int lane = threadIdx.x & 63, wave = threadIdx.x >> 6;
-    int32_t incl = wave_incl_scan(v, lane);
-    if (lane == 63) lds4[wave] = incl;
-    __syncthreads();
-    int32_t base = 0, tot = 0;
-#pragma unroll
-    for (int w = 0; w < kScanThreads / 64; ++w) {
-        int32_t s = lds4[w];
-        if (w < wave) base += s;
-        tot += s;
-    }
-    __syncthreads();
-    *total = tot;
-    return base + incl - v;
-}
-
 __global__ __launch_bounds__(kScanThreads) void k_scan_tile_sums(const int32_t *__restrict__ in, int64_t n,
                                                                  int32_t *__restrict__ tile_sums)
 {
@@ -391,7 +405,7 @@
     if (threadIdx.x == 0) *grand_total = carry;
 }
 
-__global__ __launch_bounds__(kScanThreads) void k_scan_apply(int32_t *__restrict__ data, int64_t n,
+__global__ __launch_bounds__(kScanThreads) void k_scan_apply(const int32_t *in, int32_t *data, int64_t n,
                                                              const int32_t *__restrict__ tile_sums)
 {
     __shared__ int32_t lds4[kScanThreads / 64];
@@ -401,7 +415,7 @@
 #pragma unroll
     for (int i = 0; i < kScanItems; ++i) {
         int64_t p = base + i;
-        v[i] = (p < n) ? data[p] : 0;
+        v[i] = (p < n) ? in[p] : 0;
         s += v[i];
     }
     int32_t tot;
@@ -414,97 +428,74 @@
     }
 }
 
-__global__ __launch_bounds__(kScanThreads) void k_scan_lookback(int32_t *__restrict__ data, int64_t n, uint64_t *__restrict__ state,
+__global__ __launch_bounds__(kScanThreads) void k_scan_lookback(const int32_t *in, int32_t *data, int64_t n, uint64_t *__restrict__ state,
                                                                 uint32_t *__restrict__ ticket, uint32_t epoch4, int32_t n_tiles,
                                                                 int32_t *__restrict__ host_total)
 {
     __shared__ int32_t lds4[kScanThreads / 64];
     __shared__ int32_t s_tile, s_prefix;
-    if (threadIdx.x == 0) s_tile = (int32_t)atomicAdd(ticket, 1u);
-    __syncthreads();
-    const int tile = s_tile;
+    const int tile = scan_take_tile(ticket, &s_tile);
     const int64_t base = (int64_t)tile * kScanTile + (int64_t)threadIdx.x * kScanItems;
     int32_t v[kScanItems];
-    int32_t s = 0;
 #pragma unroll
     for (int i = 0; i < kScanItems; ++i) {
         const int64_t p = base + i;
-        v[i] = (p < n) ? data[p] : 0;
-        s += v[i];
-    }
-    int32_t tot;
-    int32_t ex = block_excl_scan(s, lds4, &tot);
-    if (threadIdx.x == 0) {
-        int32_t prefix = 0;
-        if (tile > 0) {
-            __hip_atomic_store(&state[tile], ((uint64_t)(epoch4 + 1u) << 32) | (uint32_t)tot, __ATOMIC_RELAXED, __HIP_MEMORY_SCOPE_AGENT);
-            for (int p = tile - 1;; --p) {
-                uint64_t w;
-                for (;;) {
-                    w = __hip_atomic_load(&state[p], __ATOMIC_RELAXED, __HIP_MEMORY_SCOPE_AGENT);
-                    const uint32_t f = (uint32_t)(w >> 32);
-                    if (f == epoch4 + 1u || f == epoch4 + 2u) break;
-                    __builtin_amdgcn_s_sleep(2);
-                }
-                prefix += (int32_t)(uint32_t)w;
-                if ((uint32_t)(w >> 32) == epoch4 + 2u) break;
-            }
-        }
-        __hip_atomic_store(&state[tile], ((uint64_t)(epoch4 + 2u) << 32) | (uint32_t)(prefix + tot), __ATOMIC_RELAXED,
-                           __HIP_MEMORY_SCOPE_AGENT);
-        s_prefix = prefix;
-        if (tile == n_tiles - 1) {
-            data[n] = prefix + tot;
-            if (host_total) __hip_atomic_store(host_total, prefix + tot, __ATOMIC_RELAXED, __HIP_MEMORY_SCOPE_SYSTEM);
-            *ticket = 0u;
-        }
-    }
-    __syncthreads();
-    ex += s_prefix;
-#pragma unroll
-    for (int i = 0; i < kScanItems; ++i) {
-        const int64_t p = base + i;
-        if (p < n) data[p] = ex;
-        ex += v[i];
-    }
-}
-
-int exclusive_scan_i32(pfz_ctx *ctx, int32_t *data, int64_t n, LazyI32 *total)
+        v[i] = (p < n) ? in[p] : 0;
+    }
+    (void)scan_lookback_tile(v, tile, data, n, state, ticket, epoch4, n_tiles, host_total, lds4, &s_prefix);
+}
+
+int scan_single_pass(pfz_ctx *ctx, int64_t n, ScanPass *pass, bool *ok)
+{
+    const int64_t n_tiles = (n + kScanTile - 1) / kScanTile;
+    static const bool three = getenv("PFZ_SCAN3") != nullptr;
+    *ok = !three && n_tiles < (1 << 24);
+    if (!*ok) return PFZ_OK;
+    if ((size_t)n_tiles > ctx->scan_tiles) {
+        size_t cap = ctx->scan_tiles ? ctx->scan_tiles : 1024;
+        while (cap < (size_t)n_tiles) cap *= 2;
+        uint64_t *fresh = nullptr;
+        PFZ_TRY(pool_alloc(ctx, &fresh, (cap + 1) * sizeof(uint64_t)));
+        PFZ_HIP(hipMemsetAsync(fresh, 0, (cap + 1) * sizeof(uint64_t), ctx->stream));
+        if (ctx->scan_state) pool_free(ctx->scan_state);
+        ctx->scan_state = fresh;
+        ctx->scan_tiles = cap;
+        ctx->scan_epoch = 0;
+    }
+    if (ctx->scan_epoch >= (1u << 29)) {
+        PFZ_HIP(hipMemsetAsync(ctx->scan_state, 0, (ctx->scan_tiles + 1) * sizeof(uint64_t), ctx->stream));
+        ctx->scan_epoch = 0;
+    }
+    pass->state = ctx->scan_state;
+    pass->ticket = (uint32_t *)(ctx->scan_state + ctx->scan_tiles);
+    pass->epoch4 = ++ctx->scan_epoch * 4u;
+    pass->n_tiles = (int32_t)n_tiles;
+    return PFZ_OK;
+}
+
+int exclusive_scan_i32(pfz_ctx *ctx, int32_t *data, int64_t n, LazyI32 *total, const int32_t *src)
 {
     if (n <= 0) {
         PFZ_HIP(hipMemsetAsync(data, 0, sizeof(int32_t), ctx->stream));
         return total ? lazy_begin(ctx, total, data) : PFZ_OK;
     }
-    const int64_t n_tiles = (n + kScanTile - 1) / kScanTile;
-    static const bool three = getenv("PFZ_SCAN3") != nullptr;
-    if (!three && n_tiles < (1 << 24)) {
-        if ((size_t)n_tiles > ctx->scan_tiles) {
-            size_t cap = ctx->scan_tiles ? ctx->scan_tiles : 1024;
-            while (cap < (size_t)n_tiles) cap *= 2;
-            uint64_t *fresh = nullptr;
-            PFZ_TRY(pool_alloc(ctx, &fresh, (cap + 1) * sizeof(uint64_t)));
-            PFZ_HIP(hipMemsetAsync(fresh, 0, (cap + 1) * sizeof(uint64_t), ctx->stream));
-            if (ctx->scan_state) pool_free(ctx->scan_state);
-            ctx->scan_state = fresh;
-            ctx->scan_tiles = cap;
-            ctx->scan_epoch = 0;
-        }
-        if (ctx->scan_epoch >= (1u << 29)) {
-            PFZ_HIP(hipMemsetAsync(ctx->scan_state, 0, (ctx->scan_tiles + 1) * sizeof(uint64_t), ctx->stream));
-            ctx->scan_epoch = 0;
-        }
-        const uint32_t epoch4 = ++ctx->scan_epoch * 4u;
+    const int32_t *in = src ? src : data;
+    ScanPass pass;
+    bool single = false;
+    PFZ_TRY(scan_single_pass(ctx, n, &pass, &single));
+    if (single) {
         if (total) PFZ_TRY(lazy_acquire(ctx, total));
-        hipLaunchKernelGGL(k_scan_lookback, dim3((unsigned)n_tiles), dim3(kScanThreads), 0, ctx->stream, data, n, ctx->scan_state,
-                           (uint32_t *)(ctx->scan_state + ctx->scan_tiles), epoch4, (int32_t)n_tiles, total ? total->slot : nullptr);
+        hipLaunchKernelGGL(k_scan_lookback, dim3((unsigned)pass.n_tiles), dim3(kScanThreads), 0, ctx->stream, in, data, n, pass.state,
+                           pass.ticket, pass.epoch4, pass.n_tiles, total ? total->slot : nullptr);
         PFZ_HIP(hipGetLastError());
         return total ? lazy_mark(ctx, total) : PFZ_OK;
     }
+    const int64_t n_tiles = (n + kScanTile - 1) / kScanTile;
     PFZ_TRY(ensure_scratch(ctx, (size_t)n_tiles * sizeof(int32_t)));
     int32_t *tile_sums = (int32_t *)ctx->scratch;
-    hipLaunchKernelGGL(k_scan_tile_sums, dim3((unsigned)n_tiles), dim3(kScanThreads), 0, ctx->stream, data, n, tile_sums);
+    hipLaunchKernelGGL(k_scan_tile_sums, dim3((unsigned)n_tiles), dim3(kScanThreads), 0, ctx->stream, in, n, tile_sums);
     hipLaunchKernelGGL(k_scan_sums, dim3(1), dim3(kScanThreads), 0, ctx->stream, tile_sums, n_tiles, data + n);
-    hipLaunchKernelGGL(k_scan_apply, dim3((unsigned)n_tiles), dim3(kScanThreads), 0, ctx->stream, data, n, tile_sums);
+    hipLaunchKernelGGL(k_scan_apply, dim3((unsigned)n_tiles), dim3(kScanThreads), 0, ctx->stream, in, data, n, tile_sums);
     PFZ_HIP(hipGetLastError());
     return total ? lazy_begin(ctx, total, data + n) : PFZ_OK;
 }
@@ -813,7 +804,7 @@
     if (!m) return;
     if (m->ctx) (void)hipSetDevice(m->ctx->device);
     if (m->nnz_lazy.pending || m->nnz_lazy.slot) {
-        if (m->nnz_lazy.ev) (void)hipEventSynchronize(m->nnz_lazy.ev);
+        (void)pfz::lazy_wait(m->ctx, &m->nnz_lazy);
         pfz::lazy_release(m->ctx, &m->nnz_lazy);
     }
     if (m->indptr) pool_free(m->indptr);
diff --git a/polyfuzz_amd/csrc/pfz_internal.h b/polyfuzz_amd/csrc/pfz_internal.h
--- a/polyfuzz_amd/csrc/pfz_internal.h
+++ b/polyfuzz_amd/csrc/pfz_internal.h
@@ -45,6 +45,7 @@
 }
 struct K3SymState;
 
+constexpr int32_t kLazyUnset = INT32_MIN;
 struct LazyI32 {
     hipEvent_t ev = nullptr;
     int32_t *slot = nullptr;
@@ -208,6 +209,8 @@
 int lazy_begin(pfz_ctx *ctx, LazyI32 *z, const int32_t *dev);
 int lazy_acquire(pfz_ctx *ctx, LazyI32 *z);
 int lazy_mark(pfz_ctx *ctx, LazyI32 *z);
+bool lazy_ready(const LazyI32 *z);
+int lazy_wait(pfz_ctx *ctx, const LazyI32 *z);
 int lazy_get(pfz_ctx *ctx, LazyI32 *z, int32_t *out);
 void lazy_release(pfz_ctx *ctx, LazyI32 *z);
 int64_t csr_nnz(const pfz_csr *m);
@@ -241,7 +244,7 @@
 int comm_agree(pfz_comm *c, bool mine, bool *all);
 void comm_abort(pfz_comm *c);
 
-int exclusive_scan_i32(pfz_ctx *ctx, int32_t *data, int64_t n, LazyI32 *total = nullptr);
+int exclusive_scan_i32(pfz_ctx *ctx, int32_t *data, int64_t n, LazyI32 *total = nullptr, const int32_t *src = nullptr);
 
 int best_to_topn(pfz_ctx *ctx, const int32_t *d_idx, const double *d_score, int64_t n, pfz_topn *out);
 
diff --git a/polyfuzz_amd/csrc/pfz_scan.h b/polyfuzz_amd/csrc/pfz_scan.h
--- /dev/null
+++ b/polyfuzz_amd/csrc/pfz_scan.h
@@ -0,0 +1,101 @@
+#pragma once
+#include "pfz_internal.h"
+
+namespace pfz {
+
+constexpr int kScanThreads = 256;
+constexpr int kScanItems = 16;
+constexpr int kScanTile = kScanThreads * kScanItems;
+
+__device__ inline int32_t wave_incl_scan(int32_t v, int lane)
+{
+#pragma unroll
+    for (int d = 1; d < 64; d <<= 1) {
+        int32_t o = __shfl_up(v, d, 64);
+        if (lane >= d) v += o;
+    }
+    return v;
+}
+
+__device__ inline int32_t block_excl_scan(int32_t v, int32_t *lds4, int32_t *total)
+{
+    const int lane = threadIdx.x & 63, wave = threadIdx.x >> 6;
+    int32_t incl = wave_incl_scan(v, lane);
+    if (lane == 63) lds4[wave] = incl;
+    __syncthreads();
+    int32_t base = 0, tot = 0;
+#pragma unroll
+    for (int w = 0; w < kScanThreads / 64; ++w) {
+        int32_t s = lds4[w];
+        if (w < wave) base += s;
+        tot += s;
+    }
+    __syncthreads();
+    *total = tot;
+    return base + incl - v;
+}
+
+__device__ inline int scan_take_tile(uint32_t *ticket, int32_t *s_tile)
+{
+    if (threadIdx.x == 0) *s_tile = (int32_t)atomicAdd(ticket, 1u);
+    __syncthreads();
+    return *s_tile;
+}
+
+__device__ inline bool scan_lookback_tile(const int32_t (&v)[kScanItems], int tile, int32_t *out, int64_t n, uint64_t *state,
+                                          uint32_t *ticket, uint32_t epoch4, int32_t n_tiles, int32_t *host_total,
+                                          int32_t *lds4, int32_t *s_prefix)
+{
+    const int64_t base = (int64_t)tile * kScanTile + (int64_t)threadIdx.x * kScanItems;
+    int32_t s = 0;
+#pragma unroll
+    for (int i = 0; i < kScanItems; ++i) s += v[i];
+    int32_t tot;
+    int32_t ex = block_excl_scan(s, lds4, &tot);
+    bool last = false;
+    if (threadIdx.x == 0) {
+        int32_t prefix = 0;
+        if (tile > 0) {
+            __hip_atomic_store(&state[tile], ((uint64_t)(epoch4 + 1u) << 32) | (uint32_t)tot, __ATOMIC_RELAXED, __HIP_MEMORY_SCOPE_AGENT);
+            for (int p = tile - 1;; --p) {
+                uint64_t w;
+                for (;;) {
+                    w = __hip_atomic_load(&state[p], __ATOMIC_RELAXED, __HIP_MEMORY_SCOPE_AGENT);
+                    const uint32_t f = (uint32_t)(w >> 32);
+                    if (f == epoch4 + 1u || f == epoch4 + 2u) break;
+                    __builtin_amdgcn_s_sleep(2);
+                }
+                prefix += (int32_t)(uint32_t)w;
+                if ((uint32_t)(w >> 32) == epoch4 + 2u) break;
+            }
+        }
+        __hip_atomic_store(&state[tile], ((uint64_t)(epoch4 + 2u) << 32) | (uint32_t)(prefix + tot), __ATOMIC_RELAXED,
+                           __HIP_MEMORY_SCOPE_AGENT);
+        *s_prefix = prefix;
+        if (tile == n_tiles - 1) {
+            out[n] = prefix + tot;
+            if (host_total) __hip_atomic_store(host_total, prefix + tot, __ATOMIC_RELAXED, __HIP_MEMORY_SCOPE_SYSTEM);
+            *ticket = 0u;
+            last = true;
+        }
+    }
+    __syncthreads();
+    ex += *s_prefix;
+#pragma unroll
+    for (int i = 0; i < kScanItems; ++i) {
+        const int64_t p = base + i;
+        if (p < n) out[p] = ex;
+        ex += v[i];
+    }
+    return last;
+}
+
+struct ScanPass {
+    uint64_t *state = nullptr;
+    uint32_t *ticket = nullptr;
+    uint32_t epoch4 = 0;
+    int32_t n_tiles = 0;
+};
+int scan_single_pass(pfz_ctx *ctx, int64_t n, ScanPass *pass, bool *ok);
+
+}
```

Result: no change. 3619 billion, median of 6 (+0.5%).
